# ssheybani/baby-vision-curriculum

Hardware: AMD Instinct MI355X
Metric: video clips/sec (node) VideoMAE-base 16x224^2 bf16 pretraining (higher is better)
Workload: dtype bf16; 1 GPU; VideoMAE-base (ViT-B/16 encoder, 4-layer decoder), 16x224x224 clips, tubelet 2, 90% tube mask, full training step (fwd + MSE + bwd + GradScaler + SGD-Nesterov); clips_per_gpu=256, global_batch=256, parallelism=dp1, weights=random init N(0,0.02), seed 0

## Files before the change

baby-vision-curriculum_amd/_lib.py:

```python
import ctypes
import os
import sys

_HERE = os.path.dirname(os.path.abspath(__file__))
LIB_PATH = os.environ.get("BVC_LIB_PATH") or os.path.join(_HERE, "libbvc_hip.so")

c_void_p, c_int, c_int64, c_float, c_char_p = ctypes.c_void_p, ctypes.c_int, ctypes.c_int64, ctypes.c_float, ctypes.c_char_p
c_double = ctypes.c_double


class BvcError(RuntimeError):
    pass


class VideoMAEConfigC(ctypes.Structure):
    _fields_ = [(n, c_int) for n in (
        "image_size", "patch_size", "num_channels", "num_frames", "tubelet_size",
        "hidden_size", "num_hidden_layers", "num_attention_heads", "intermediate_size",
        "decoder_hidden_size", "decoder_num_hidden_layers", "decoder_num_attention_heads",
        "decoder_intermediate_size")] + [("layer_norm_eps", c_float), ("decoder_norm_eps", c_float),
                                         ("norm_pix_loss", c_int)]


class VitConfigC(ctypes.Structure):
# ... 160 lines not shown
    "bvc_dropout_mask_host": (c_int, [ctypes.c_uint64, ctypes.c_uint64, c_int, c_int, c_int, c_int, c_float, c_void_p]),
    "bvc_videomae_cls_set_drop": (c_int, [c_void_p, ctypes.POINTER(BranchDropC), c_int, c_void_p]),
    "bvc_videomae_encoder_set_drop": (c_int, [c_void_p, ctypes.POINTER(BranchDropC), c_int, c_void_p]),
    "bvc_vit_set_drop": (c_int, [c_void_p, ctypes.POINTER(BranchDropC), c_int, c_void_p]),
    "bvc_predictor_set_drop": (c_int, [c_void_p, ctypes.POINTER(BranchDropC), c_int, c_void_p]),
    "bvc_op_attention_fwd": (c_int, [c_void_p, c_void_p, c_void_p, c_int, c_int, c_int, c_int, c_void_p]),
    "bvc_op_attention_bwd": (c_int, [c_void_p, c_void_p, c_void_p, c_void_p, c_void_p, c_void_p, c_int, c_int, c_int, c_int, c_void_p]),
    "bvc_op_attention_bwd_part": (c_int, [c_void_p, c_void_p, c_void_p, c_void_p, c_void_p, c_void_p, c_int, c_int, c_int, c_int, c_int, c_void_p]),
    "bvc_op_attention_width": (c_int, [c_int]),
    "bvc_op_attention_fwd_scaled": (c_int, [c_void_p, c_void_p, c_void_p, c_int, c_int, c_int, c_int, ctypes.c_float, c_void_p]),
    "bvc_op_attention_bwd_scaled": (c_int, [c_void_p, c_void_p, c_void_p, c_void_p, c_void_p, c_void_p, c_int, c_int, c_int, c_int,
                                            ctypes.c_float, c_void_p]),
    "bvc_op_attention_probs": (c_int, [c_void_p, c_void_p, c_void_p, c_int, c_int, c_int, c_int, ctypes.c_float, c_void_p]),
    "bvc_op_layernorm_fwd": (c_int, [c_void_p, c_int, c_int, c_int, c_void_p, c_void_p, c_void_p, c_void_p, c_void_p,
                                     c_int, c_int, c_float, c_void_p]),
    "bvc_op_layernorm_bwd": (c_int, [c_void_p, c_void_p, c_int, c_int, c_int, c_void_p, c_void_p, c_void_p, c_void_p,
                                     c_int, c_void_p, c_void_p, c_void_p, c_void_p, c_int, c_int, c_void_p]),
    "bvc_op_layernorm_bwd_workspace": (c_int64, [c_int, c_int]),
    "bvc_op_colsum_bf16": (c_int, [c_void_p, c_int, c_int, c_int, c_float, c_void_p, c_void_p, c_void_p]),
    "bvc_op_colsum_f32": (c_int, [c_void_p, c_int, c_int, c_int, c_int, c_int, c_void_p, c_void_p]),
    "bvc_op_cast_bf16": (c_int, [c_void_p, c_void_p, c_int64, c_void_p]),
    "bvc_op_row_normalize": (c_int, [c_void_p, c_void_p, c_void_p, c_int, c_int, c_float, c_void_p]),
    "bvc_op_row_normalize_bwd": (c_int, [c_void_p, c_void_p, c_void_p, c_void_p, c_int, c_int, c_void_p]),
    "bvc_op_nce_finalize": (c_int, [c_void_p, c_int, c_float, c_int64, c_void_p, c_void_p, c_void_p]),
    "bvc_op_sgd_step": (c_int, [c_void_p, c_void_p, c_void_p, c_int64, c_float, c_float, c_float, c_float, c_int, c_int, c_int,
                                c_void_p, c_void_p, c_int, c_void_p, c_void_p]),
    "bvc_videomae_shadow": (c_int, [c_void_p, c_int, ctypes.POINTER(c_void_p), ctypes.POINTER(c_int64)]),
    "bvc_vit_shadow": (c_int, [c_void_p, c_int, ctypes.POINTER(c_void_p), ctypes.POINTER(c_int64)]),
    "bvc_predictor_shadow": (c_int, [c_void_p, c_int, ctypes.POINTER(c_void_p), ctypes.POINTER(c_int64)]),
    "bvc_op_adam_prepare": (c_int, [c_void_p, c_double, c_double, c_double, c_void_p, c_void_p]),
    "bvc_op_adam_step": (c_int, [c_void_p, c_void_p, c_void_p, c_void_p, c_int64, c_double, c_double, c_double, c_double, c_double,
                                 c_int, c_int, c_void_p, c_void_p, c_void_p, c_int, c_void_p, c_void_p]),
    "bvc_op_row_ln_selected": (c_int, [c_int, c_int, c_int, c_int]),
    "bvc_op_sgd_step_segments": (c_int, [c_void_p, c_void_p, c_void_p, c_int64, c_void_p, c_void_p, c_void_p, c_int, c_void_p, c_void_p, c_void_p,
                                         c_int, c_void_p, c_void_p]),
    "bvc_op_adam_step_segments": (c_int, [c_void_p, c_void_p, c_void_p, c_void_p, c_int64, c_void_p, c_void_p, c_void_p, c_int, c_void_p, c_void_p,
                                          c_void_p, c_void_p, c_void_p, c_int, c_void_p, c_void_p]),
    "bvc_op_nonfinite_check": (c_int, [c_void_p, c_int64, c_void_p, c_void_p]),
    "bvc_op_mask_index": (c_int, [c_void_p, c_int, c_int, c_int, c_int, c_void_p, c_void_p, c_void_p, c_void_p]),
    "bvc_op_dual_mask_index": (c_int, [c_void_p, c_void_p, c_int, c_int, c_int, c_int, c_void_p, c_void_p, c_void_p, c_void_p]),
    "bvc_op_gather_patches": (c_int, [c_void_p, c_void_p, c_void_p, c_int, c_int, c_int, c_int, c_int, c_int, c_int, c_int, c_void_p]),
    "bvc_op_pixel_labels": (c_int, [c_void_p, c_void_p, c_void_p, c_int, c_int, c_int, c_int, c_int, c_int, c_int, c_int, c_int, c_void_p]),
    "bvc_comm_unique_id": (c_int, [c_void_p]),
    "bvc_comm_init": (c_int, [c_int, c_int, c_void_p, ctypes.POINTER(c_void_p)]),
    "bvc_comm_destroy": (c_int, [c_void_p]),
    "bvc_comm_stream": (c_void_p, [c_void_p]),
    "bvc_comm_rank": (c_int, [c_void_p]),
    "bvc_comm_world": (c_int, [c_void_p]),
    "bvc_comm_library": (c_char_p, []),
    "bvc_allreduce_bucket": (c_int, [c_void_p, c_void_p, c_int64, c_int, c_void_p]),
    "bvc_comm_wait": (c_int, [c_void_p, c_void_p]),
    "bvc_allgather": (c_int, [c_void_p, c_void_p, c_void_p, c_int64, c_void_p]),
    "bvc_allreduce": (c_int, [c_void_p, c_void_p, c_int64, c_int, c_void_p]),
    "bvc_broadcast": (c_int, [c_void_p, c_void_p, c_int64, c_int, c_void_p]),
}

_lib = None

_det_flag = False
_det_pushed = False


def use_deterministic_algorithms(mode):
    global _det_flag
    _det_flag = bool(mode)
    lib()
# ... 51 lines not shown
```

baby-vision-curriculum_amd/csrc/gemm.h:

```cpp
#pragma once
#include "common.h"
#include "dropgate.h"
#include "../../include/bvc.h"

namespace bvc {

enum GemmLayout { GEMM_NT = BVC_GEMM_NT, GEMM_NN = BVC_GEMM_NN, GEMM_TN = BVC_GEMM_TN };

enum GemmEpilogue {
    EPI_F32 = BVC_EPI_F32,
    EPI_BF16 = BVC_EPI_BF16,
    EPI_GELU = BVC_EPI_GELU,
    EPI_RESID = BVC_EPI_RESID,
    EPI_POS = BVC_EPI_POS,
    EPI_E2D = BVC_EPI_E2D,
    EPI_LOSS = BVC_EPI_LOSS,
    EPI_DGELU = BVC_EPI_DGELU,
    EPI_F32_BF16 = BVC_EPI_F32_BF16,
    EPI_RELU = BVC_EPI_RELU,
    EPI_DRELU = BVC_EPI_DRELU,
    EPI_NCE = BVC_EPI_NCE,
    EPI_NCE_BWD = BVC_EPI_NCE_BWD,
    EPI_RESID_LN = BVC_EPI_RESID_LN,
    EPI_DLN = BVC_EPI_DLN,
    EPI_RESID_GATE = BVC_EPI_RESID_GATE
};

using GemmProblem = bvc_gemm_desc;

constexpr int kMaxGroup = 4;

struct Options { int gemm8 = 0; int dw_overlap = 0; int row_ln = 0; int row_stagger = 1; int deterministic = 0; int head_pad = 0; int dec_tail = 1; };
Options& options();

float* det_scratch(size_t floats, hipStream_t stream);
size_t det_scratch_bytes();
int det_scratch_release();

struct DryRun { bool on = false; char name[160] = ""; };
DryRun& dry_run();

int launch_gemm(const GemmProblem* probs, int nprob, GemmLayout layout, int tile_cfg, hipStream_t stream, int stages = -1);

int launch_gemm_gate(const GemmProblem& p, const Gate& gate, int tile_cfg, hipStream_t stream);

int gemm_num_tiles(const GemmProblem& p, int tile_cfg);
int gemm_pick_tile(const GemmProblem* probs, int nprob, int tile_cfg);
bool gemm_row_ln_ok(int M, int N, int K);
constexpr size_t kRowLnPartFloats = 512 * 2 * 384;

}
```

baby-vision-curriculum_amd/csrc/gemm.hip:

```cpp
#include <stdio.h>
#include <stdlib.h>
#include <string.h>

#include <algorithm>
#include <mutex>
#include <vector>

#include "gemm_tile.h"

namespace bvc {

Options& options() {
    static Options o;
    return o;
}
DryRun& dry_run() {
    static thread_local DryRun d;
    return d;
}

template <int BM, int BN, bool AT, bool BT, int NS, int LB = 2, bool EARLY_ = true>
__global__ __launch_bounds__(256, LB) void gemm_kernel(const GemmGroup g) {
    constexpr bool DET = false;
#include "gemm_kernel_body.inc"
// ... 298 lines not shown
    BVC_REQUIRE(p.A && p.B && p.C && p.resid, "launch_gemm_gate: null operand, output or residual");
    BVC_REQUIRE(gate.rows >= 1 && (double)p.M * p.N < 4398046511104.0, "launch_gemm_gate: bad gate (rows per sample %d) or more than 2^42 elements", gate.rows);
    const int cfg = gemm_pick_tile(&p, 1, tile_cfg);
    GemmGroup g;
    g.nprob = 1;
    g.bal_units = g.bal_lb = g.bal_tiles = 0;
    g.accum = 0;
    g.stagger = 0;
    g.dbg = 0;
    const int total = tiles_for(p, cfg);
    for (int i = 0; i < kMaxGroup; ++i) { g.prob[i] = p; g.panel[i] = pick_panel(p, cfg, GEMM_NT); g.tile_start[i] = i == 0 ? 0 : total; }
    g.tile_start[kMaxGroup] = total;
    switch (cfg) {
        case 0: return launch_gate_one<128, 128>(g, gate, total, stream);
        case 1: return launch_gate_one<128, 64>(g, gate, total, stream);
        default: return launch_gate_one<64, 64>(g, gate, total, stream);
    }
}

int launch_gemm(const GemmProblem* probs, int nprob, GemmLayout layout, int tile_cfg, hipStream_t stream, int stages) {
    BVC_REQUIRE(nprob >= 1 && nprob <= kMaxGroup, "launch_gemm: nprob %d out of range", nprob);
    for (int i = 0; i < nprob; ++i)
        BVC_REQUIRE(probs[i].epi != EPI_RESID_GATE, "launch_gemm: BVC_EPI_RESID_GATE needs its gate (bvc_op_gemm_gate / a context with bvc_*_set_drop)");
    static thread_local bool skip_g8 = false;
    bool auto_g8 = false;
    if (probs[0].epi == EPI_RESID_LN || probs[0].epi == EPI_DLN) {
        const GemmProblem& p = probs[0];
        BVC_REQUIRE(nprob == 1 && (tile_cfg < 0 || tile_cfg == 12), "launch_gemm: the LayerNorm epilogues take one problem on tile config 12");
        BVC_REQUIRE(gemm_row_ln_ok(p.M, p.N, p.K) && p.ldc == p.N && p.split_k == 1 && p.a_bytes < 0x80000000u && p.b_bytes < 0x80000000u,
                    "launch_gemm: the LayerNorm epilogues need N == ldc == 384, K %% 64 == 0, operands below 2 GiB (M=%d N=%d K=%d)", p.M, p.N, p.K);
        BVC_REQUIRE(p.C && p.C2 && p.ln_mean && p.ln_rstd && p.ln_gamma, "launch_gemm: LayerNorm epilogue with a null output / statistic / scale");
        if (p.epi == EPI_RESID_LN) BVC_REQUIRE(layout == GEMM_NT && p.resid && p.ln_beta, "launch_gemm: RESID_LN is an NT product with a residual and a LayerNorm bias");
        if (p.epi == EPI_DLN) BVC_REQUIRE(layout == GEMM_NN && p.ln_x && p.ln_part && p.ln_dgamma && p.ln_dbeta, "launch_gemm: DLN is an NN product with the LayerNorm input, partial scratch and parameter gradients");
        if (p.seg_rows != 0)
            BVC_REQUIRE(p.seg_rows > 0 && p.seg_rows % 128 == 0 && p.M % p.seg_rows == 0 && p.seg_off >= 0 && p.seg_stride > 0 &&
                            (long long)p.seg_off + p.seg_rows <= (long long)p.seg_stride,
                        "launch_gemm: bad segment map (seg_rows %d: a multiple of 128 that divides M = %d; seg_off %d + seg_rows <= seg_stride %d)",
                        p.seg_rows, p.M, p.seg_off, p.seg_stride);
        tile_cfg = 12;
    } else {
        for (int i = 0; i < nprob; ++i)
            BVC_REQUIRE(probs[i].seg_rows == 0, "launch_gemm: a segment map (seg_rows %d) exists for BVC_EPI_RESID_LN / BVC_EPI_DLN only", probs[i].seg_rows);
    }
    if (tile_cfg < 0 && stages < 0 && nprob == 1 && options().gemm8 >= 0 && probs[0].epi == EPI_BF16 && gemm_as_ok(probs[0], layout) &&
        (options().gemm8 > 0 || probs[0].M >= 16384) && BVC_EXP_ENV("BVC_GEMM_NO_AS") == nullptr)
        return launch_gemm_as(probs[0], layout, 0, stream);
    if (tile_cfg < 0 && stages < 0 && !skip_g8) {
        const int g8 = pick_gemm8(probs, nprob, layout);
        if (g8 > 0) { tile_cfg = g8; auto_g8 = true; }
    }
    if (tile_cfg >= 15 && tile_cfg <= 18) {
        BVC_REQUIRE(nprob == 1, "launch_gemm: tile configs 15 - 18 take one problem");
        const int rc = launch_gemm_as(probs[0], layout, tile_cfg - 15, stream);
        BVC_REQUIRE(rc != 1, "launch_gemm: tile configs 15 - 18 (A-stationary kernel) take NT products with K = 384, N %% 128 == 0, BF16 / GELU epilogues");
        return rc;
    }
    if ((tile_cfg >= 3 && tile_cfg <= 5) || tile_cfg == 8) {
#ifdef BVC_EXPERIMENTS
        BVC_REQUIRE(nprob == 1 && layout == GEMM_NT, "launch_gemm: tile configs 3-5 (32-deep K steps) are NT, one problem");
        BVC_REQUIRE(!options().deterministic || probs[0].split_k == 1, "launch_gemm: tile configs 3-5 have no deterministic split-K form");
        return launch_gemm_big_nt(probs[0], tile_cfg, stream);
#else
        BVC_REQUIRE(false, "launch_gemm: tile configs 3-5 / 8 exist only in a -DBVC_EXPERIMENTS build (csrc/experiments/gemm_big.hip)");
#endif
    }
    bool accum = false;
// ... 143 lines not shown
```

baby-vision-curriculum_amd/csrc/gemm8.hip:

```cpp
#include <stdio.h>
#include <stdlib.h>

#include <type_traits>

#include "gemm_tile.h"
#include "rowops.h"

namespace bvc {

namespace {

typedef __attribute__((ext_vector_type(4))) unsigned int u32x4;

#ifndef BVC_G8_ST_AUX
#define BVC_G8_ST_AUX 0
#endif
#ifndef BVC_G8_ROW_ST_AUX
#define BVC_G8_ROW_ST_AUX 0
#endif
constexpr uint32_t kInvalidBase = 0x80000000u;

struct Unit {
    int pi, m0, n0, kt0, nkt, split, tile;
};
// ... 39 lines not shown
        const int w = lid - split * ntiles;
        if (tiles_n > tiles_m) { tm = w % tiles_m; tn = w / tiles_m; } else { tm = w / tiles_n; tn = w % tiles_n; }
    } else {
        split = lid % p.split_k;
        const int tl = lid / p.split_k;
        const bool m_fast = tiles_n > tiles_m;
        tm = m_fast ? tl % tiles_m : tl / tiles_n;
        tn = m_fast ? tl / tiles_m : tl % tiles_n;
    }
    const int nt_all = (p.K + 63) / 64;
    int per = (nt_all + p.split_k - 1) / p.split_k;
    per = (per + 1) & ~1;
    int kt0 = split * per;
    if (g.bal_units > 0) {
        kt0 = split * g.bal_lb;
        per = tail ? (nt_all - kt0 + 1) & ~1 : g.bal_lb;
    }
    u.pi = pi;
    u.m0 = __builtin_amdgcn_readfirstlane(tm * BM);
    u.n0 = __builtin_amdgcn_readfirstlane(tn * BN);
    u.kt0 = __builtin_amdgcn_readfirstlane(kt0);
    u.nkt = __builtin_amdgcn_readfirstlane(per);
    u.split = __builtin_amdgcn_readfirstlane(split);
    u.tile = __builtin_amdgcn_readfirstlane(tm * tiles_n + tn);
}

}

template <int BM, int BN, bool AT, bool BT, int EC>
__global__ __launch_bounds__(512, 1) void gemm8_kernel(const GemmGroup g, const int total_units) {
    extern __shared__ __attribute__((aligned(16))) char smem[];
    static_assert(BM == 256 || (BM == 128 && BN == 384), "128-row tiles: the 128 x 384 geometry only");
    static_assert(BN == 256 || BN == 128 || (BN == 384 && BM == 128), "column tiles of 256 / 128, or 384 with 128 rows");
    static_assert((EC == 4 || EC == 5) == (BM == 128 && !AT), "row epilogues (EC 4 / 5) are the k-contiguous-A instantiations of the 128 x 384 tile, and only they");
    static_assert(BM == 256 || EC == 4 || EC == 5 || (AT && BT && (EC == 2 || EC == 6)), "128 x 384 with transposed A: weight gradients");
    static_assert(EC != 6 || (AT && BT), "EC 6 (deterministic weight gradients) is a TN product");
    static_assert(EC != 4 || !BT, "EC 4 (residual + LayerNorm forward) is an NT product");
    constexpr int A_BYTES = BM * 64 * 2, B_BYTES = BN * 64 * 2, TILE = A_BYTES + B_BYTES;
    constexpr int WMR = BM / 2;
    constexpr int WN = BN / 4, TN = WN / 16, TM = WMR / 16, TMH = TM / 2;
    constexpr int NB = BN / 64, NBH = BN / 128, NAH = BM / 128;
    constexpr int n0c = AT ? NBH : (NB == 6 ? 3 : NB < 2 ? NB : 2), n1c = AT ? NAH : NB - n0c, n2c = AT ? NBH : BM / 128, n3c = AT ? NAH : BM / 128;
    constexpr int RT = BM / 128;
    constexpr int KMAX = (n0c > 2 || n1c > 2 || n2c > 2 || n3c > 2) ? 3 : 2;
    constexpr int PT = n0c + n1c + n2c + n3c;
#ifdef BVC_G8_DMA_LATE
    constexpr bool LATE = true;
#else
    constexpr bool LATE = false;
#endif
    constexpr int PAR_BYTES = EC == 4 ? 3 * BN * 4 : EC == 5 ? BN * 4 : 0, STAT_OFF = PAR_BYTES, COL_OFF = STAT_OFF + 4096;
    constexpr int CPR = BN == 384 ? 8 : WN / 8;
    constexpr int NSIDE = TM * (16 / (64 / CPR));
    static_assert(PT + 2 * NSIDE < 64, "vmcnt is a 6-bit counter");
    constexpr int WP = AT ? PT : n3c + n0c + n1c;
    constexpr int W1 = LATE ? n0c + n1c + n2c : PT;
    constexpr int W3 = LATE ? (AT ? n2c + n3c + n0c : n3c + n0c) : WP;

    const int tid = threadIdx.x, lane = tid & 63;
    const int wave = __builtin_amdgcn_readfirstlane(tid >> 6);
    const int wm = wave >> 2, wn = wave & 3;

    const int xcd = blockIdx.x & 7, slot_id = blockIdx.x >> 3, nslots = gridDim.x >> 3;
    const int xq = total_units >> 3, xr = total_units & 7;
    const int x_lo = xcd < xr ? xcd * (xq + 1) : xr * (xq + 1) + (xcd - xr) * xq;
    const int x_hi = x_lo + xq + (xcd < xr ? 1 : 0);
    int uid = x_lo + slot_id, u_step = nslots, u_hi = x_hi;
    if (EC == 2 && g.bal_units > 0) {
        u_step = 1;
        if (uid < x_hi) {
            u_hi = uid + 1;
        } else {
            const int J = xcd * nslots - x_lo + (uid - x_hi), I = 8 * nslots - g.bal_units;
            uid = g.bal_units + (J * g.bal_tiles) / I;
            u_hi = g.bal_units + ((J + 1) * g.bal_tiles) / I;
        }
    }
    if (uid >= u_hi) {
        if constexpr (EC == 5) {
            float* pr = g.prob[0].ln_part + (size_t)blockIdx.x * 2 * BN;
            for (int i = tid; i < 2 * BN; i += 512) pr[i] = 0.f;
        }
        return;
    }
    if constexpr (EC == 4 || EC == 5) {
        const int cnt = x_hi - x_lo, r = cnt % nslots, nmax = (cnt + nslots - 1) / nslots;
        int num = 0, den = 1;
        if (r > 0 && slot_id >= r) { num = slot_id - r + 1; den = nslots - r + 1; }
        else if (r == 0 && nmax >= 4) { num = slot_id; den = 2 * nslots; }
        const int quanta = __builtin_amdgcn_readfirstlane((int)((long long)g.stagger * num / den));
        for (int i = 0; i < quanta / 127; ++i) __builtin_amdgcn_s_sleep(127);
    }
    if (BVC_DBG(g, 1024) && (slot_id & 1)) {
        for (int i = 0; i < ((g.dbg >> 12) & 63); ++i) __builtin_amdgcn_s_sleep(127);
    }

    Unit su;
    decode_unit<BM, BN>(g, uid, su);
    int s_uid = uid, s_kt = 0;
    bool s_valid = true;
    __amdgpu_buffer_rsrc_t s_ra, s_rb;
    uint32_t s_la, s_lb, s_baseA, s_baseB, s_strideA, s_strideB;
    auto s_problem = [&]() {
        const GemmProblem& p = g.prob[su.pi];
        s_ra = make_rsrc(p.A, p.a_bytes);
        s_rb = make_rsrc(p.B, p.b_bytes);
        if constexpr (!AT) {
            const int r = 8 * wave + (lane >> 3);
            s_la = (uint32_t)((r * p.lda + (((lane & 7) ^ swz_rows(r)) << 3)) * 2);
            s_strideA = (uint32_t)(64 * p.lda * 2);
        } else {
            const int kr = 4 * wave + (lane >> 4);
            s_la = (uint32_t)((kr * p.lda + (((lane & 15) ^ swz_tr<128>(kr)) << 3)) * 2);
            s_strideA = (uint32_t)(32 * p.lda * 2);
        }
        if constexpr (!BT) {
            const int r = 8 * wave + (lane >> 3);
            s_lb = (uint32_t)((r * p.ldb + (((lane & 7) ^ swz_rows(r)) << 3)) * 2);
// ... 57 lines not shown
            else { if constexpr (K < n3c) load_a(ra_, BM == 256 ? (K == 0 ? 1 : 3) : 1); }
        } else {
            if constexpr (GI == 0) { if constexpr (K < NBH) load_b(rb_, 2 * K); }
            else if constexpr (GI == 1) { if constexpr (K < NAH) load_a(ra_, 2 * K); }
            else if constexpr (GI == 2) { if constexpr (K < NBH) load_b(rb_, 2 * K + 1); }
            else { if constexpr (K < NAH) load_a(ra_, 2 * K + 1); }
        }
        if constexpr (GI == 3 && K == KMAX - 1) s_advance();
    };
    auto stage_group = [&](auto gi_, char* buf) {
        stage_one(gi_, I0{}, buf); stage_one(gi_, I1{}, buf);
        if constexpr (KMAX == 3) stage_one(gi_, I2{}, buf);
    };
    auto stage_phase = [&](auto q_, auto k_, char* cur, char* oth) {
        constexpr int Q = decltype(q_)::value;
        if constexpr (Q == 0) stage_one(I2{}, k_, oth);
        else if constexpr (Q == 1) stage_one(I3{}, k_, oth);
        else if constexpr (Q == 2) stage_one(I0{}, k_, cur);
        else stage_one(I1{}, k_, cur);
    };

    char* const buf0 = smem;
    char* const buf1 = smem + TILE;
    constexpr int PARK = BN == 384 ? 16 * 48 * 4 : 16 * WN * 4;
    AS3 char* const wl = (AS3 char*)smem + 2 * TILE + wave * PARK;

    if constexpr (EC == 0) {
        const GemmProblem& p0 = g.prob[0];
        AS3 float* lbias = (AS3 float*)((AS3 char*)smem + 2 * TILE);
        const int npad = ((p0.N + BN - 1) / BN) * BN;
        for (int i = tid; i < npad; i += 512) lbias[i] = (p0.bias && i < p0.N) ? p0.bias[i] : 0.f;
        __syncthreads();
    }
    if constexpr (EC == 4 || EC == 5) {
        const GemmProblem& p0 = g.prob[0];
        AS3 float* lpar = (AS3 float*)((AS3 char*)smem + 2 * TILE);
        for (int i = tid; i < BN; i += 512) {
            if constexpr (EC == 4) {
                lpar[i] = p0.bias ? p0.bias[i] : 0.f;
                lpar[BN + i] = p0.ln_gamma[i];
                lpar[2 * BN + i] = p0.ln_beta[i];
            } else {
                lpar[i] = p0.ln_gamma[i];
            }
        }
        if constexpr (EC == 5) {
            AS3 float* lcol = (AS3 float*)((AS3 char*)smem + 2 * TILE + COL_OFF);
            for (int i = tid; i < 8 * 2 * WN; i += 512) lcol[i] = 0.f;
        }
        __syncthreads();
    }
    s_problem();
    s_ktile();
    stage_group(I0{}, buf0); stage_group(I1{}, buf0); stage_group(I2{}, buf0); stage_group(I3{}, buf0);
    stage_group(I0{}, buf1); stage_group(I1{}, buf1);
    wait_vmcnt<WP>();
    asm volatile("s_barrier" ::: "memory");
#ifndef BVC_G8_NO_STAGGER
    if (wm == 1) asm volatile("s_barrier" ::: "memory");
#endif

    Unit cu;
    decode_unit<BM, BN>(g, uid, cu);
    int after_epi = 0;


    while (true) {
        const GemmProblem& p = g.prob[cu.pi];
        f32x4 acc[TM][TN];
#pragma unroll
        for (int i = 0; i < TM; ++i)
#pragma unroll
            for (int j = 0; j < TN; ++j) acc[i][j] = f32x4{0.f, 0.f, 0.f, 0.f};
        float rsum[2] = {0.f, 0.f};
        const bool do_rowsum = (EC == 2 || EC == 6) && p.rowsum != nullptr && cu.n0 == 0;

        auto ktile = [&](auto rs_, char* cur, char* oth) {
            constexpr bool RS = decltype(rs_)::value;
            const char* la = cur;
            const char* lb = cur + A_BYTES;
            if constexpr (!AT) {
// ... 95 lines not shown
                                case 2: a = af[2]; break;
                                default: a = af[3]; break;
                            }
                        } else {
                            a = wn == 0 ? af[0] : af[1];
                        }
                        union { bf16x8 v; uint32_t u[4]; } w;
                        w.v = a;
                        float t0 = 0.f, t1 = 0.f;
#pragma unroll
                        for (int e = 0; e < 4; ++e) {
                            t0 += __uint_as_float(w.u[e] << 16);
                            t1 += __uint_as_float(w.u[e] & 0xffff0000u);
                        }
                        rsum[mh] += t0 + t1;
                    }
                    __builtin_amdgcn_s_setprio(0);
                    __builtin_amdgcn_sched_barrier(0);
                    asm volatile("s_barrier" ::: "memory");
                };
                phase(I0{}); phase(I1{}); phase(I2{}); phase(I3{});
            }
            after_epi = 0;
        };

        for (int kt = 0; kt < cu.nkt; kt += 2) {
            ktile(std::bool_constant<EC == 2 || EC == 6>{}, buf0, buf1);
            ktile(std::bool_constant<EC == 2 || EC == 6>{}, buf1, buf0);
        }

        const int m0 = cu.m0, n0 = cu.n0;
        const int epi = p.epi, Mrows = p.M, Ncols = p.N, ldc = p.ldc;
        int seg_shift = 0;
        if constexpr (EC == 4 || EC == 5) {
            if (p.seg_rows > 0) {
                const int upc = p.seg_rows >> 7, u = m0 >> 7, c = u / upc;
                seg_shift = __builtin_amdgcn_readfirstlane(c * p.seg_stride + p.seg_off + ((u - c * upc) << 7) - m0);
            }
        }
        const float alpha = p.alpha_dev ? p.alpha * p.alpha_dev[0] : p.alpha;
        constexpr int UNITS = WN / 4;
        constexpr int RPU = 64 / CPR;
        constexpr int U = 16 / RPU;
        static_assert(NSIDE == TM * U, "epilogue geometry");
        int nstores = 0;
        constexpr uint32_t kDrop = 0xFFFFFFF0u;
        auto park = [&](int i) {
            const int row = lane & 15;
#pragma unroll
            for (int j = 0; j < TN; ++j) {
                const int unit = (4 * j + (lane >> 4)) ^ (row & (UNITS - 1));
                *reinterpret_cast<AS3 f32x4*>(wl + row * (WN * 4) + unit * 16) = acc[i][j];
            }
        };
        const bool atomic = p.split_k > 1 || g.accum != 0;
        if constexpr (EC == 0) {
            const __amdgpu_buffer_rsrc_t rc = make_rsrc(p.C, BVC_DBG(g, 1) ? 0u : kDrop);
            const __amdgpu_buffer_rsrc_t rc2 = make_rsrc(p.C2 ? p.C2 : p.C, BVC_DBG(g, 1) ? 0u : kDrop);
            const AS3 float* lbias = (const AS3 float*)((AS3 char*)smem + 2 * TILE);
            const int q4 = lane >> 4;
            f32x4 bj[TN];
#pragma unroll
            for (int j = 0; j < TN; ++j) {
                const int nb = n0 + wn * WN + 16 * j + 4 * q4;
                bj[j] = *reinterpret_cast<const AS3 f32x4*>(lbias + nb);
            }
            const bool two_out = epi == EPI_GELU;
// ... 85 lines not shown
            issue(I0{});
            wait_vmcnt<0>();
#pragma unroll
            for (int j = 0; j < TN; ++j) asm volatile("" : "+v"(rs[0][j]));
            tile(I0{}); tile(I1{}); tile(I2{}); tile(I3{});
            asm volatile("s_waitcnt lgkmcnt(0)\n\ts_barrier" ::: "memory");
#pragma unroll
            for (int i = 0; i < TM; ++i) {
                asm volatile("" ::: "memory");
                const AS3 f32x4* sp = reinterpret_cast<const AS3 f32x4*>(lstat + (wm * 64 + 16 * i + r16) * 8);
                const f32x4 a = sp[0], b = sp[1];
                const float mean = ((a[0] + a[2]) + (b[0] + b[2])) * (1.f / BN);
                const float d0 = a[0] * (1.f / WN) - mean, d1 = a[2] * (1.f / WN) - mean, d2 = b[0] * (1.f / WN) - mean, d3 = b[2] * (1.f / WN) - mean;
                const float m2 = ((a[1] + a[3]) + (b[1] + b[3])) + (float)WN * ((d0 * d0 + d1 * d1) + (d2 * d2 + d3 * d3));
                const float rstd = rsqrtf(m2 * (1.f / BN) + eps);
                const int m = m0 + 32 * i + 16 * wm + r16;
                if (wn == 0 && q4 == 0) {
                    __builtin_amdgcn_raw_buffer_store_b32(__float_as_uint(mean), rmu, (uint32_t)m * 4u, 0, 0);
                    __builtin_amdgcn_raw_buffer_store_b32(__float_as_uint(rstd), rrs, (uint32_t)m * 4u, 0, 0);
                }
                const uint32_t o2 = ((uint32_t)m * (uint32_t)BN + (uint32_t)(wn * WN + 16 * (q4 & 1) + 8 * (q4 >> 1))) * 2u;
#pragma unroll
                for (int jp = 0; jp < TN / 2; ++jp) {
                    const f32x4 ga = *reinterpret_cast<const AS3 f32x4*>(lpar + BN + cw + 32 * jp), gb = *reinterpret_cast<const AS3 f32x4*>(lpar + BN + cw + 32 * jp + 16);
                    const f32x4 ba = *reinterpret_cast<const AS3 f32x4*>(lpar + 2 * BN + cw + 32 * jp), bb = *reinterpret_cast<const AS3 f32x4*>(lpar + 2 * BN + cw + 32 * jp + 16);
                    const f32x4 ya = ((acc[i][2 * jp] - mean) * rstd) * ga + ba;
                    const f32x4 yb = ((acc[i][2 * jp + 1] - mean) * rstd) * gb + bb;
                    const uint32_t a0 = pack2bf(ya[0], ya[1]), a1 = pack2bf(ya[2], ya[3]), b0 = pack2bf(yb[0], yb[1]), b1 = pack2bf(yb[2], yb[3]);
                    const auto s0 = __builtin_amdgcn_permlane16_swap(a0, b0, false, false);
                    const auto s1 = __builtin_amdgcn_permlane16_swap(a1, b1, false, false);
                    __builtin_amdgcn_raw_buffer_store_b128(u32x4{s0[0], s1[0], s0[1], s1[1]}, rc2, o2 + 64u * jp, 0, BVC_G8_ROW_ST_AUX);
                }
            }
        } else if constexpr (EC == 5) {
            const uint32_t ext = (uint32_t)Mrows * (uint32_t)(BN * 4);
            const __amdgpu_buffer_rsrc_t rx = make_rsrc(p.ln_x, ext), rd = make_rsrc(reinterpret_cast<float*>(p.C) + (size_t)seg_shift * BN, ext), rc2 = make_rsrc(p.C2, ext / 2);
            const __amdgpu_buffer_rsrc_t rmu = make_rsrc(p.ln_mean, (uint32_t)Mrows * 4u), rrs = make_rsrc(p.ln_rstd, (uint32_t)Mrows * 4u);
            const AS3 float* lpar = (const AS3 float*)((AS3 char*)smem + 2 * TILE);
            AS3 float* lstat = (AS3 float*)((AS3 char*)smem + 2 * TILE + STAT_OFF);
            AS3 float* lcol = (AS3 float*)((AS3 char*)smem + 2 * TILE + COL_OFF) + wave * 2 * WN;
            const int q4 = lane >> 4, r16 = lane & 15;
            const int cw = wn * WN + 4 * q4;
            const int mrow = m0 + 16 * wm + r16;
            const uint32_t obase = (uint32_t)mrow * (uint32_t)(BN * 4) + (uint32_t)cw * 4u;
            const uint32_t o2base = ((uint32_t)mrow * (uint32_t)BN + (uint32_t)(wn * WN + 16 * (q4 & 1) + 8 * (q4 >> 1))) * 2u;
            f32x4 xr[2][TN], dr[TN];
            float mu[2], rsd[2];
            auto issue = [&](auto i_) {
                constexpr int i = decltype(i_)::value;
                mu[i & 1] = __uint_as_float(__builtin_amdgcn_raw_buffer_load_b32(rmu, (uint32_t)(mrow + 32 * i) * 4u, 0, 0));
                rsd[i & 1] = __uint_as_float(__builtin_amdgcn_raw_buffer_load_b32(rrs, (uint32_t)(mrow + 32 * i) * 4u, 0, 0));
#pragma unroll
                for (int j = 0; j < TN; ++j)
                    xr[i & 1][j] = __builtin_bit_cast(f32x4, __builtin_amdgcn_raw_buffer_load_b128(rx, obase + (uint32_t)(i * 32 * BN * 4 + 64 * j), 0, 0));
            };
            auto tile = [&](auto i_) {
                constexpr int i = decltype(i_)::value, b = i & 1;
                __builtin_amdgcn_sched_barrier(0);
#pragma unroll
                for (int j = 0; j < TN; ++j)
                    dr[j] = __builtin_bit_cast(f32x4, __builtin_amdgcn_raw_buffer_load_b128(rd, obase + (uint32_t)(i * 32 * BN * 4 + 64 * j), 0, 0));
                if constexpr (i + 1 < TM) issue(std::integral_constant<int, i + 1>{});
                __builtin_amdgcn_sched_barrier(0);
                float s1 = 0.f, s2 = 0.f;
#pragma unroll
                for (int j = 0; j < TN; ++j) {
                    const f32x4 gam = *reinterpret_cast<const AS3 f32x4*>(lpar + cw + 16 * j);
                    const f32x4 gv = acc[i][j] * alpha;
                    const f32x4 xh = (xr[b][j] - mu[b]) * rsd[b];
                    const f32x4 gg = gv * gam;
                    f32x4 tg = gv * xh, tb = gv;
                    s1 += (gg[0] + gg[1]) + (gg[2] + gg[3]);
                    const f32x4 gx = gg * xh;
                    s2 += (gx[0] + gx[1]) + (gx[2] + gx[3]);
                    xr[b][j] = xh;
                    acc[i][j] = gg;
#pragma unroll
                    for (int e = 0; e < 4; ++e) {
                        tg[e] = row16_sum(tg[e]);
                        tb[e] = row16_sum(tb[e]);
                    }
                    if (r16 == 0) {
                        AS3 f32x4* cg = reinterpret_cast<AS3 f32x4*>(lcol + 16 * j + 4 * q4);
                        AS3 f32x4* cb = reinterpret_cast<AS3 f32x4*>(lcol + WN + 16 * j + 4 * q4);
                        *cg = *cg + tg;
                        *cb = *cb + tb;
                    }
                }
                s1 += __shfl_xor(s1, 16, 64);
                s1 += __shfl_xor(s1, 32, 64);
                s2 += __shfl_xor(s2, 16, 64);
                s2 += __shfl_xor(s2, 32, 64);
                if (q4 == 0) *reinterpret_cast<AS3 f32x2*>(lstat + ((wm * 64 + 16 * i + r16) * 4 + wn) * 2) = f32x2{s1, s2};
                asm volatile("s_waitcnt lgkmcnt(0)\n\ts_barrier" ::: "memory");
                const AS3 f32x4* sp = reinterpret_cast<const AS3 f32x4*>(lstat + (wm * 64 + 16 * i + r16) * 8);
                const f32x4 sa = sp[0], sb = sp[1];
                const float c1 = ((sa[0] + sa[2]) + (sb[0] + sb[2])) * (1.f / BN), c2 = ((sa[1] + sa[3]) + (sb[1] + sb[3])) * (1.f / BN);
#pragma unroll
                for (int j = 0; j < TN; ++j) {
                    acc[i][j] = ((acc[i][j] - c1) - xr[b][j] * c2) * rsd[b] + dr[j];
                    __builtin_amdgcn_raw_buffer_store_b128(__builtin_bit_cast(u32x4, acc[i][j]), rd, obase + (uint32_t)(i * 32 * BN * 4 + 64 * j), 0, BVC_G8_ROW_ST_AUX);
                }
#pragma unroll
                for (int jp = 0; jp < TN / 2; ++jp) {
                    const f32x4 ya = acc[i][2 * jp], yb = acc[i][2 * jp + 1];
                    const uint32_t a0 = pack2bf(ya[0], ya[1]), a1 = pack2bf(ya[2], ya[3]), b0 = pack2bf(yb[0], yb[1]), b1 = pack2bf(yb[2], yb[3]);
                    const auto w0 = __builtin_amdgcn_permlane16_swap(a0, b0, false, false);
                    const auto w1 = __builtin_amdgcn_permlane16_swap(a1, b1, false, false);
                    __builtin_amdgcn_raw_buffer_store_b128(u32x4{w0[0], w1[0], w0[1], w1[1]}, rc2, o2base + (uint32_t)(i * 32 * BN * 2 + 64 * jp), 0, BVC_G8_ROW_ST_AUX);
                }
            };
            issue(I0{});
            wait_vmcnt<0>();
            asm volatile("" : "+v"(mu[0]), "+v"(rsd[0]));
#pragma unroll
            for (int j = 0; j < TN; ++j) asm volatile("" : "+v"(xr[0][j]));
            tile(I0{}); tile(I1{}); tile(I2{}); tile(I3{});
        } else if constexpr (BN == 384) {
            const __amdgpu_buffer_rsrc_t rca = make_rsrc(p.C, kDrop);
            const __amdgpu_buffer_rsrc_t rsl = make_rsrc(EC == 6 && atomic ? p.partial + (size_t)cu.split * Mrows * Ncols : p.C, kDrop);
#pragma unroll
            for (int i = 0; i < TM; ++i) {
#pragma unroll
                for (int ps = 0; ps < 2; ++ps) {
                    const int prow = lane & 15;
#pragma unroll
                    for (int jj = 0; jj < 3; ++jj)
                        *reinterpret_cast<AS3 f32x4*>(wl + prow * 192 + (4 * jj + (lane >> 4)) * 16) = acc[i][3 * ps + jj];
#pragma unroll
                    for (int t = 0; t < 16 * 48 / 64; ++t) {
                        const int idx = t * 64 + lane;
                        const int row = idx / 48, col = idx % 48;
                        const int m = m0 + wm * WMR + 16 * i + row, n = n0 + wn * WN + 48 * ps + col;
                        const float v = *reinterpret_cast<const AS3 float*>(wl + row * 192 + col * 4) * alpha;
// ... 154 lines not shown
            }
            }
            if (EC == 1 && epi == EPI_LOSS) {
                const float w = wave_sum(sumsq);
                float* red = reinterpret_cast<float*>(smem + 2 * TILE);
                if (lane == 0) red[wave * (16 * WN)] = w;
                asm volatile("s_waitcnt lgkmcnt(0)\n\ts_barrier" ::: "memory");
                asm volatile("s_barrier" ::: "memory");
                if (tid == 0) {
                    float s = 0.f;
#pragma unroll
                    for (int q = 0; q < 8; ++q) s += red[q * (16 * WN)];
                    p.partial[cu.tile] = s;
                }
            }
        }
        if (do_rowsum) {
#pragma unroll
            for (int mh = 0; mh < 2; ++mh) {
                float v = rsum[mh];
                v += __shfl_xor(v, 16, 64);
                v += __shfl_xor(v, 32, 64);
                const int m = m0 + wm * WMR + 16 * (TMH * mh + wn) + lane;
                if constexpr (EC == 6) {
                    if (wn < TMH && (lane >> 4) == 0 && m < p.M) p.ln_part[(size_t)cu.split * p.M + m] = v * alpha;
                } else {
                    if (wn < TMH && (lane >> 4) == 0 && m < p.M) atomicAdd(p.rowsum + m, v * alpha);
                }
            }
        }
        uid += u_step;
        if (uid >= u_hi) break;
        decode_unit<BM, BN>(g, uid, cu);
        after_epi = (EC == 4 || EC == 5) ? -1 : (((EC == 2 || EC == 6) && atomic) || BN == 384) ? 0 : EC == 0 ? nstores : -1;
    }
    wait_vmcnt<0>();
#ifndef BVC_G8_NO_STAGGER
    if (wm == 0) asm volatile("s_barrier" ::: "memory");
#endif
    if constexpr (EC == 5) {
        __syncthreads();
        const AS3 float* lcol = (const AS3 float*)((AS3 char*)smem + 2 * TILE + COL_OFF);
        float* pr = g.prob[0].ln_part + (size_t)blockIdx.x * 2 * BN;
        for (int c = tid; c < 2 * BN; c += 512) {
            const int which = c / BN, col = c % BN, w = col / WN, cc = col % WN;
            pr[c] = lcol[(w * 2 + which) * WN + cc] + lcol[((4 + w) * 2 + which) * WN + cc];
        }
    }
}

static int g8_ncu() {
    static int ncu = 0;
    if (ncu == 0) {
        int dev = 0;
        hipDeviceProp_t prop;
        if (hipGetDevice(&dev) != hipSuccess || hipGetDeviceProperties(&prop, dev) != hipSuccess) return 256;
        ncu = prop.multiProcessorCount > 0 ? (prop.multiProcessorCount / 8) * 8 : 256;
        if (ncu < 8) ncu = 8;
    }
    return ncu;
}

static bool plan_balance(GemmGroup& g, int bm, int bn, int total, int ncu) {
    if (BVC_EXP_ENV("BVC_G8_NO_BALANCE") != nullptr) return false;
    const int S = g.prob[0].split_k, nt = (g.prob[0].K + 63) / 64;
    if ((S < 2 && !g.accum) || total >= ncu || total % S != 0) return false;
    for (int i = 0; i < g.nprob; ++i) {
        const GemmProblem& p = g.prob[i];
        if (p.split_k != S || (p.K + 63) / 64 != nt || p.epi != EPI_F32) return false;
        if (g.tile_start[i] % S != 0 || g.panel[i] == 0) return false;
    }
    const int T = total / S, I = ncu - total, q = (T + I - 1) / I;
    double e = 6.0, c = 1.0;
    if (const char* v = BVC_EXP_ENV("BVC_G8_BALANCE_EPI")) e = atof(v);
    if (const char* v = BVC_EXP_ENV("BVC_G8_BALANCE_TAIL")) c = atof(v);
    const double lt = ((double)nt / S - (q - 1) * e) / (q * c + 1.0 / S);
    if (lt < 2.0) return false;
    const int per = (((nt + S - 1) / S) + 1) & ~1;
    const int lb = (int)((nt - lt) / S) & ~1;
    if (lb < 8 || nt - S * lb < 2 || lb > 0.95 * per) return false;
    g.bal_units = total;
    g.bal_lb = lb;
    g.bal_tiles = T;
    (void)bm; (void)bn;
    return true;
}

template <int BM, int BN, bool AT, bool BT, int EC>
static int launch_gemm8_one(const GemmGroup& g_in, int total, hipStream_t stream) {
    constexpr size_t lds = 2 * (size_t)(BM + BN) * 64 * 2 + (EC == 0 ? (size_t)32768 : EC == 4 ? (size_t)(3 * BN * 4 + 4096) : EC == 5 ? (size_t)(BN * 4 + 4096 + 8 * 2 * (BN / 4) * 4) :
                                                              BN == 384 ? (size_t)8 * 16 * 48 * 4 : (size_t)8 * 16 * (BN / 4) * 4);
    static_assert(lds <= 160 * 1024, "LDS per CU");
    if (dry_run().on) {
        snprintf(dry_run().name, sizeof(dry_run().name), "bvc::gemm8_kernel<%d, %d, %s, %s, %d>", BM, BN, AT ? "true" : "false", BT ? "true" : "false", EC);
        return BVC_OK;
    }
    static bool attr_set = false;
    if (!attr_set) {
        BVC_CHECK_HIP(hipFuncSetAttribute(reinterpret_cast<const void*>(&gemm8_kernel<BM, BN, AT, BT, EC>),
                                          hipFuncAttributeMaxDynamicSharedMemorySize, (int)lds));
        attr_set = true;
    }
    const int ncu = g8_ncu();
    GemmGroup g = g_in;
    int grid = total < ncu ? ((total + 7) / 8) * 8 : ncu;
    if constexpr (EC == 2) {
        if (plan_balance(g, BM, BN, total, ncu)) grid = ncu;
    }
    if constexpr (EC == 4 || EC == 5) {
        const double us = 1.45 * ((g.prob[0].K + 63) / 64) + (EC == 4 ? 23.0 : 32.0);
        g.stagger = options().row_stagger && total > ncu ? (int)(us * 33.0) : 0;
    }
    hipLaunchKernelGGL((gemm8_kernel<BM, BN, AT, BT, EC>), dim3(grid), dim3(512), lds, stream, g, total);
    BVC_CHECK_HIP(hipGetLastError());
    (void)0;
    if constexpr (EC == 5)
        return launch_ln_param_reduce(g.prob[0].ln_part, grid, BN, g.prob[0].ln_dgamma, g.prob[0].ln_dbeta, stream);
    return BVC_OK;
}

static int epi_class(int epi, GemmLayout layout) {
    if (layout == GEMM_TN) return epi == EPI_F32 ? 2 : -1;
    if (epi == EPI_RESID_LN) return layout == GEMM_NT ? 4 : -1;
    if (epi == EPI_DLN) return layout == GEMM_NN ? 5 : -1;
    switch (epi) {
        case EPI_BF16: case EPI_GELU: case EPI_RELU: return 0;
        case EPI_DGELU: case EPI_DRELU: return 3;
        case EPI_F32: case EPI_RESID: case EPI_POS: case EPI_E2D: case EPI_LOSS: case EPI_F32_BF16: return 1;
        default: return -1;
    }
}

int launch_gemm8(const GemmGroup& g, GemmLayout layout, int bn, hipStream_t stream, bool det) {
    const int total = g.tile_start[g.nprob];
    int ec = -2;
    for (int i = 0; i < g.nprob; ++i) {
        const GemmProblem& p = g.prob[i];
        const int c = epi_class(p.epi, layout);
        if (c < 0 || (ec != -2 && c != ec)) return 1;
        ec = c;
        if (p.a_bytes >= kInvalidBase || p.b_bytes >= kInvalidBase) return 1;
        if (layout != GEMM_TN && (p.split_k != 1 || p.K % 64 != 0)) return 1;
        if (layout == GEMM_TN && p.split_k > 1 && p.epi != EPI_F32) return 1;
        if (p.rowsum && layout != GEMM_TN) return 1;
        if (c == 0 && (g.nprob != 1 || (size_t)((p.N + bn - 1) / bn) * bn * 4 > (size_t)32768)) return 1;
    }
    if (total <= 0) return 1;
#define BVC_G8(BN_, AT_, BT_, EC_) return launch_gemm8_one<256, BN_, AT_, BT_, EC_>(g, total, stream)
    if (bn == 384) {
        if (layout == GEMM_TN) return ec != 2 ? 1 : det ? launch_gemm8_one<128, 384, true, true, 6>(g, total, stream)
                                                        : launch_gemm8_one<128, 384, true, true, 2>(g, total, stream);
        const GemmProblem& p = g.prob[0];
        if (g.nprob != 1 || p.N != 384 || p.ldc != 384 || (double)p.M * 1536.0 >= 4294000000.0) return 1;
        if (ec == 4 && layout == GEMM_NT) return launch_gemm8_one<128, 384, false, false, 4>(g, total, stream);
        if (ec == 5 && layout == GEMM_NN) return launch_gemm8_one<128, 384, false, true, 5>(g, total, stream);
        return 1;
    }
    if (ec >= 4) return 1;
    if (layout == GEMM_NT) {
        if (ec == 0) { if (bn == 256) BVC_G8(256, false, false, 0); else BVC_G8(128, false, false, 0); }
        if (ec == 3) { if (bn == 256) BVC_G8(256, false, false, 3); else BVC_G8(128, false, false, 3); }
        if (ec == 1) { if (bn == 256) BVC_G8(256, false, false, 1); else BVC_G8(128, false, false, 1); }
    } else if (layout == GEMM_NN) {
        if (ec == 0) { if (bn == 256) BVC_G8(256, false, true, 0); else BVC_G8(128, false, true, 0); }
        if (ec == 3) { if (bn == 256) BVC_G8(256, false, true, 3); else BVC_G8(128, false, true, 3); }
        if (ec == 1) { if (bn == 256) BVC_G8(256, false, true, 1); else BVC_G8(128, false, true, 1); }
    } else if (det) {
        if (bn == 256) BVC_G8(256, true, true, 6); else BVC_G8(128, true, true, 6);
    } else {
        if (bn == 256) BVC_G8(256, true, true, 2); else BVC_G8(128, true, true, 2);
    }
#undef BVC_G8
    return 1;
}

}
```

baby-vision-curriculum_amd/csrc/rowops.h:

```cpp
#pragma once
#include "common.h"
#include "dropgate.h"

namespace bvc {

struct RowMap { int rin, rout, roff; };
static inline RowMap identity_rows() { return RowMap{0, 0, 0}; }

struct PatchGeom { int T, C, H, W, ts, ps; };

struct PixelSrc {
    const void* ptr;
    int is_u8;
    float mean[4], stdv[4];
};
static inline PixelSrc pixels_f32(const float* p) { return PixelSrc{p, 0, {0, 0, 0, 0}, {1, 1, 1, 1}}; }

int launch_ln_fwd(const float* x, RowMap rm, const float* gamma, const float* beta, bf16_t* y, float* mean, float* rstd,
                  int M, int D, float eps, hipStream_t s, float* y32 = nullptr);
size_t ln_bwd_workspace_floats(int M, int D);
size_t ln_bwd_workspace_floats_upto(int Mmax, int D);
int launch_ln_bwd(const bf16_t* dy, const float* x, RowMap rm, const float* mean, const float* rstd, const float* gamma,
                  float* dres, int accumulate, bf16_t* dres_bf, float* dgamma, float* dbeta, float* part, int M, int D, hipStream_t s,
                  const Gate* gate = nullptr,
                  bool compact_x = false);
int launch_ln_param_reduce(const float* part, int nblk, int D, float* dgamma, float* dbeta, hipStream_t s);
int launch_colsum_bf16(const bf16_t* X, int M, int N, int ld, float alpha, float* out, hipStream_t s);
int launch_colsum_bf16_scaled(const bf16_t* X, int M, int N, int ld, float alpha, const float* alpha_dev, float* out, hipStream_t s);
int launch_colsum_f32(const float* X, RowMap rm, int M, int D, float* out, hipStream_t s);
int launch_token_mean(const float* x, int B, int N, int D, float* out, hipStream_t s);
int launch_token_mean_bwd(const float* dmean, int B, int N, int D, float* dx, hipStream_t s);
int launch_fcnorm_bwd_bcast(const float* dy, const float* p, const float* mean, const float* rstd, const float* gamma, float* dres,
                            bf16_t* dres_bf, float* dgamma, float* dbeta, int B, int N, int D, hipStream_t s, const Gate* gate = nullptr);
int launch_dropout_mask(const Gate& gate, size_t n, uint8_t* out, hipStream_t s);
void dropout_mask_host(const Gate& gate, size_t n, uint8_t* out);
int launch_cast_bf16(const float* in, bf16_t* out, size_t n, hipStream_t s);
int launch_gather_rows_bf16(const float* in, RowMap rm, bf16_t* out, int M, int D, hipStream_t s);
int launch_mask_index(const uint8_t* mask, int B, int L, int nvis, int nmask, int* vis_idx, int* msk_idx, int* status, hipStream_t s);
int launch_dual_mask_index(const uint8_t* mask, const uint8_t* decode, int B, int L, int nvis, int ndec, int* vis_idx, int* dec_idx,
                           int* status, hipStream_t s);
int launch_gather_patches(PixelSrc clip, const int* vis_idx, bf16_t* A, int B, int nvis, PatchGeom pg, hipStream_t s);
int launch_labels(PixelSrc clip, const int* dec_idx, float* labels, int B, int ndec, PatchGeom pg, int norm_pix, hipStream_t s);
int launch_fill_masked(float* xfull, const float* mask_token, const float* pos, const int* dec_idx, int B, int Ld, int nvis,
                       int ndec, int D, hipStream_t s);
int launch_sgd_step(float* p, float* g, float* buf, size_t n, float lr, float momentum, float dampening, float wd, int nesterov,
                    int first, int maximize, const float* grad_scale, const float* found_inf, int write_grad, bf16_t* shadow,
                    hipStream_t s);
int launch_adam_prep(float* state, double lr, double beta1, double beta2, const float* found_inf, hipStream_t s);
int launch_adam_step(float* p, float* g, float* m, float* v, size_t n, double lr, double beta1, double beta2, double eps, double wd,
                     int decoupled, int maximize, const float* state, const float* grad_scale, const float* found_inf, int write_grad,
                     bf16_t* shadow, hipStream_t s);
int launch_sgd_step_segments(float* p, float* g, float* buf, int64_t n, const int64_t* seg_start, const int* seg_group, const int* blk_seg,
                             int nseg, const bvc_sgd_groups* groups, const float* grad_scale, const float* found_inf, int write_grad,
                             bf16_t* shadow, hipStream_t s);
int launch_adam_step_segments(float* p, float* g, float* m, float* v, int64_t n, const int64_t* seg_start, const int* seg_group,
                              const int* blk_seg, int nseg, const bvc_adam_groups* groups, float* state, double* hyper_dev,
                              const float* grad_scale, const float* found_inf, int write_grad, bf16_t* shadow, hipStream_t s);
int launch_pad_heads(const bf16_t* wqkv, const float* bqkv, const bf16_t* wo, bf16_t* wqkv_p, float* bqkv_p, bf16_t* wo_p, int D, int H,
                     int hd, int hdp, hipStream_t s);
int launch_unpad_head_grads(const float* gwqkv_p, const float* gbqkv_p, const float* gwo_p, float* gwqkv, float* gbqkv, float* gwo, int D,
                            int H, int hd, int hdp, hipStream_t s);
int launch_nonfinite_check(const float* x, size_t n, float* found_inf, hipStream_t s);
int launch_row_normalize(const float* f, bf16_t* fn, float* inv, int n, int p, float eps, hipStream_t s);
int launch_row_normalize_bwd(const float* f, const float* inv, const float* dfn, float* df, int n, int p, hipStream_t s);
int launch_nce_finalize(const float* partial, int ntiles, float inv_t, double npos, float* loss, float* stats, hipStream_t s);
int launch_target_select(const float* h, const int* idx, float* out, int nsets, int B, int Np, int L, int D, float eps, hipStream_t s);
int launch_pred_assemble(const float* xe, const float* mask_token, const float* pos, const int* idx_pred, float* X, int nsets, int B,
                         int Nc, int Np, int D, hipStream_t s);
int launch_pred_ctx_grad(const float* dX, bf16_t* dxe, int nsets, int B, int Nc, int Np, int D, hipStream_t s);
int smooth_l1_blocks(size_t n);
int launch_smooth_l1_fwd(const float* z, const float* h, size_t n, float* partial, float* loss, hipStream_t s);
int launch_smooth_l1_bwd(const float* z, const float* h, const float* gout, size_t n, float* dz, hipStream_t s);
int launch_ema(float* k, const float* q, size_t n, float m, hipStream_t s);
int launch_iota_mod(int* idx, int n, int L, hipStream_t s);
int launch_loss_finalize(const float* partial, int n, double count, const int* status, float* loss, hipStream_t s);

}
// ... 1 lines not shown
```

baby-vision-curriculum_amd/csrc/rowops.hip:

```cpp
#include "rowops.h"
#include "gemm.h"

#include <algorithm>

namespace bvc {

constexpr int kMaxChunks = 4;
constexpr int kWideChunks = 6;

__device__ __forceinline__ int map_row(int m, RowMap rm) {
    return rm.rin > 0 ? (m / rm.rin) * rm.rout + rm.roff + (m % rm.rin) : m;
}

template <int LPR>
__device__ __forceinline__ float row_sum(float v) {
#pragma unroll
    for (int o = LPR / 2; o > 0; o >>= 1) v += __shfl_xor(v, o, 64);
    return v;
}

template <int LPR, int NC>
__global__ __launch_bounds__(256) void ln_fwd_kernel(const float* __restrict__ x, RowMap rm, const float* __restrict__ gamma,
                                                     const float* __restrict__ beta, bf16_t* __restrict__ y, float* __restrict__ y32,
                                                     float* __restrict__ mean, float* __restrict__ rstd, int M, int D, float eps) {
// ... 231 lines not shown
    const int lane = threadIdx.x & 63, wave = threadIdx.x >> 6;
    const int col = (blockIdx.x * 64 + lane) * 8;
    float acc[8] = {0, 0, 0, 0, 0, 0, 0, 0};
    const int r0 = blockIdx.y * RB, r1 = min(M, r0 + RB);
    if (col < N) {
        for (int m = r0 + wave; m < r1; m += 4) {
            const bf16x8 v = *reinterpret_cast<const bf16x8*>(X + (size_t)m * ld + col);
#pragma unroll
            for (int e = 0; e < 8; ++e) acc[e] += bf2f((bf16_t)v[e]);
        }
    }
#pragma unroll
    for (int e = 0; e < 8; ++e) red[wave][lane * 8 + e] = acc[e];
    __syncthreads();
    for (int c = threadIdx.x; c < 512; c += 256) {
        const int n = blockIdx.x * 512 + c;
        if (n < N) {
            const float v = (alpha_dev ? alpha * alpha_dev[0] : alpha) * ((red[0][c] + red[1][c]) + (red[2][c] + red[3][c]));
            if constexpr (DET) out[(size_t)blockIdx.y * N + n] = v;
            else atomicAdd(out + n, v);
        }
    }
}
__global__ __launch_bounds__(256) void colsum_bf16_kernel(const bf16_t* __restrict__ X, int M, int N, int ld, float alpha,
                                                          const float* __restrict__ alpha_dev, float* __restrict__ out, int RB) {
    colsum_bf16_body<false>(X, M, N, ld, alpha, alpha_dev, out, RB);
}
__global__ __launch_bounds__(256) void colsum_bf16_det_kernel(const bf16_t* __restrict__ X, int M, int N, int ld, float alpha,
                                                              const float* __restrict__ alpha_dev, float* __restrict__ part, int RB) {
    colsum_bf16_body<true>(X, M, N, ld, alpha, alpha_dev, part, RB);
}

template <bool DET>
__device__ __forceinline__ void colsum_f32_body(const float* __restrict__ X, RowMap rm, int M, int D, float* __restrict__ out, int RB) {
    __shared__ float red[4][256];
    const int lane = threadIdx.x & 63, wave = threadIdx.x >> 6;
    const int col = (blockIdx.x * 64 + lane) * 4;
    f32x4 acc = {0, 0, 0, 0};
    const int r0 = blockIdx.y * RB, r1 = min(M, r0 + RB);
    if (col < D)
        for (int m = r0 + wave; m < r1; m += 4)
            acc += *reinterpret_cast<const f32x4*>(X + (size_t)map_row(m, rm) * D + col);
#pragma unroll
    for (int e = 0; e < 4; ++e) red[wave][lane * 4 + e] = acc[e];
    __syncthreads();
    const int c = threadIdx.x;
    const int n = blockIdx.x * 256 + c;
    if constexpr (DET) {
        if (n < D) out[(size_t)blockIdx.y * D + n] = (red[0][c] + red[1][c]) + (red[2][c] + red[3][c]);
    } else {
        if (n < D) atomicAdd(out + n, (red[0][c] + red[1][c]) + (red[2][c] + red[3][c]));
    }
}
__global__ __launch_bounds__(256) void colsum_f32_kernel(const float* __restrict__ X, RowMap rm, int M, int D,
                                                         float* __restrict__ out, int RB) {
    colsum_f32_body<false>(X, rm, M, D, out, RB);
}
__global__ __launch_bounds__(256) void colsum_f32_det_kernel(const float* __restrict__ X, RowMap rm, int M, int D,
                                                             float* __restrict__ part, int RB) {
    colsum_f32_body<true>(X, rm, M, D, part, RB);
}

__global__ __launch_bounds__(256) void token_mean_kernel(const float* __restrict__ x, int N, int D, float* __restrict__ out) {
    __shared__ float red[16][64];
    const int cg = threadIdx.x & 15, rp = threadIdx.x >> 4;
    const int col = blockIdx.x * 64 + cg * 4;
    const float* xb = x + (size_t)blockIdx.y * N * D;
    f32x4 acc = {0, 0, 0, 0};
    if (col < D)
        for (int m = rp; m < N; m += 16) acc += *reinterpret_cast<const f32x4*>(xb + (size_t)m * D + col);
#pragma unroll
    for (int e = 0; e < 4; ++e) red[rp][cg * 4 + e] = acc[e];
    __syncthreads();
    if (threadIdx.x < 64) {
        float t = 0.f;
#pragma unroll
        for (int r = 0; r < 16; ++r) t += red[r][threadIdx.x];
        const int n = blockIdx.x * 64 + threadIdx.x;
        if (n < D) out[(size_t)blockIdx.y * D + n] = t / (float)N;
    }
}

__global__ void token_mean_bwd_kernel(const float* __restrict__ dmean, float* __restrict__ dx, int N, int D, size_t total4) {
    const size_t i = (size_t)blockIdx.x * blockDim.x + threadIdx.x;
    if (i >= total4) return;
    const size_t e = i * 4;
    const int d = (int)(e % D);
    const size_t b = e / ((size_t)N * D);
    f32x4 g = *reinterpret_cast<const f32x4*>(dmean + b * D + d);
    const float inv = 1.f / (float)N;
    g *= inv;
    *reinterpret_cast<f32x4*>(dx + e) = g;
}
// ... 332 lines not shown
#pragma unroll
    for (int i = 0; i < 3; ++i) {
        const int c = l3 + i;
        mr[i] = (c == 0 || c == 3) ? mu[0] : (c == 1 || c == 4) ? mu[1] : mu[2];
        rr[i] = (c == 0 || c == 3) ? rinv[0] : (c == 1 || c == 4) ? rinv[1] : rinv[2];
    }
    __builtin_amdgcn_fence(__ATOMIC_RELEASE, "wavefront");
    __builtin_amdgcn_wave_barrier();
    __builtin_amdgcn_fence(__ATOMIC_ACQUIRE, "wavefront");
    float* out = labels + (size_t)m * CE;
#pragma unroll
    for (int k = 0; k < CE / 256; ++k) {
        const int o = lane * 4 + 256 * k;
        f32x4 r;
#pragma unroll
        for (int j = 0; j < 4; ++j) {
            const int t = o + j, e = t / 3, c = t - 3 * e;
            r[j] = (buf[c * E + e] - mr[(k + j) % 3]) * rr[(k + j) % 3];
        }
        *reinterpret_cast<f32x4*>(out + o) = r;
    }
}

__global__ void fill_masked_kernel(float* __restrict__ xfull, const float* __restrict__ mask_token, const float* __restrict__ pos,
                                   const int* __restrict__ dec_idx, int B, int Ld, int nvis, int ndec, int D) {
    const size_t i = (size_t)blockIdx.x * blockDim.x + threadIdx.x;
    const int nch = D >> 2;
    if (i >= (size_t)B * ndec * nch) return;
    const int m = (int)(i / nch), c = (int)(i % nch);
    const int b = m / ndec, j = m % ndec;
    const f32x4 mt = reinterpret_cast<const f32x4*>(mask_token)[c];
    const f32x4 pe = reinterpret_cast<const f32x4*>(pos + (size_t)dec_idx[m] * D)[c];
    reinterpret_cast<f32x4*>(xfull + ((size_t)b * Ld + nvis + j) * D)[c] = mt + pe;
}

__global__ __launch_bounds__(256) void loss_finalize_kernel(const float* __restrict__ partial, int n, double count,
                                                            const int* __restrict__ status, float* __restrict__ loss) {
    __shared__ double red[256];
    double s = 0.0;
    for (int i = threadIdx.x; i < n; i += 256) s += (double)partial[i];
    red[threadIdx.x] = s;
    __syncthreads();
    for (int o = 128; o > 0; o >>= 1) {
        if (threadIdx.x < o) red[threadIdx.x] += red[threadIdx.x + o];
        __syncthreads();
    }
    if (threadIdx.x == 0) *loss = (status && *status) ? __int_as_float(0x7fc00000) : (float)(red[0] / count);
}

template <int NC>
__global__ __launch_bounds__(256) void target_select_kernel(const float* __restrict__ h, const int* __restrict__ idx,
                                                            float* __restrict__ out, int rows, int B, int Np, int L, int D, float eps) {
    const int lane = threadIdx.x & 63, m = blockIdx.x * 4 + (threadIdx.x >> 6);
    if (m >= rows) return;
    const int b = (m / Np) % B;
    const f32x4* xr = reinterpret_cast<const f32x4*>(h + ((size_t)b * L + idx[m]) * D);
    const int nch = D >> 2;
    f32x4 v[NC];
    float s = 0.f;
#pragma unroll
    for (int i = 0; i < NC; ++i) {
        const int c = lane + 64 * i;
        if (c < nch) { v[i] = xr[c]; s += (v[i][0] + v[i][1]) + (v[i][2] + v[i][3]); }
    }
    const float mu = wave_sum(s) / D;
    float q = 0.f;
// ... 523 lines not shown
        float* mid = nullptr;
        if (const size_t f = det_rows_mid_floats(nblk, 2 * D)) {
            mid = det_scratch(f, s);
            if (!mid) return BVC_ERR_HIP;
        }
        return launch_det_rows_reduce(part, nblk, 2 * D, D, dgamma, dbeta, mid, s);
    }
    hipLaunchKernelGGL(ln_param_reduce_kernel, dim3((2 * D + 255) / 256, (nblk + 15) / 16), dim3(256), 0, s, part, nblk, D, dgamma, dbeta);
    BVC_CHECK_HIP(hipGetLastError());
    return BVC_OK;
}

int launch_colsum_bf16_scaled(const bf16_t* X, int M, int N, int ld, float alpha, const float* alpha_dev, float* out, hipStream_t s) {
    BVC_REQUIRE(N % 8 == 0 && ld % 8 == 0, "colsum_bf16: N and ld must be multiples of 8");
    const int RB = M >= 16384 ? 256 : 64;
    if (options().deterministic) {
        const int nrb = (M + RB - 1) / RB;
        if (nrb <= 0) return BVC_OK;
        float* part = det_scratch((size_t)nrb * N + det_rows_mid_floats(nrb, N), s);
        if (!part) return BVC_ERR_HIP;
        hipLaunchKernelGGL(colsum_bf16_det_kernel, dim3((N + 511) / 512, nrb), dim3(256), 0, s, X, M, N, ld, alpha, alpha_dev, part, RB);
        BVC_CHECK_HIP(hipGetLastError());
        return launch_det_rows_reduce(part, nrb, N, N, out, out, part + (size_t)nrb * N, s);
    }
    hipLaunchKernelGGL(colsum_bf16_kernel, dim3((N + 511) / 512, (M + RB - 1) / RB), dim3(256), 0, s, X, M, N, ld, alpha, alpha_dev, out, RB);
    BVC_CHECK_HIP(hipGetLastError());
    return BVC_OK;
}

int launch_colsum_bf16(const bf16_t* X, int M, int N, int ld, float alpha, float* out, hipStream_t s) {
    return launch_colsum_bf16_scaled(X, M, N, ld, alpha, nullptr, out, s);
}

int launch_colsum_f32(const float* X, RowMap rm, int M, int D, float* out, hipStream_t s) {
    BVC_REQUIRE(D % 4 == 0, "colsum_f32: D must be a multiple of 4");
    const int RB = 256;
    if (options().deterministic) {
        const int nrb = (M + RB - 1) / RB;
        if (nrb <= 0) return BVC_OK;
        float* part = det_scratch((size_t)nrb * D + det_rows_mid_floats(nrb, D), s);
        if (!part) return BVC_ERR_HIP;
        hipLaunchKernelGGL(colsum_f32_det_kernel, dim3((D + 255) / 256, nrb), dim3(256), 0, s, X, rm, M, D, part, RB);
        BVC_CHECK_HIP(hipGetLastError());
        return launch_det_rows_reduce(part, nrb, D, D, out, out, part + (size_t)nrb * D, s);
    }
    hipLaunchKernelGGL(colsum_f32_kernel, dim3((D + 255) / 256, (M + RB - 1) / RB), dim3(256), 0, s, X, rm, M, D, out, RB);
    BVC_CHECK_HIP(hipGetLastError());
    return BVC_OK;
}

int launch_token_mean(const float* x, int B, int N, int D, float* out, hipStream_t s) {
    BVC_REQUIRE(D % 4 == 0, "token_mean: D must be a multiple of 4");
    hipLaunchKernelGGL(token_mean_kernel, dim3((D + 63) / 64, B), dim3(256), 0, s, x, N, D, out);
    BVC_CHECK_HIP(hipGetLastError());
    return BVC_OK;
}

int launch_token_mean_bwd(const float* dmean, int B, int N, int D, float* dx, hipStream_t s) {
    BVC_REQUIRE(D % 4 == 0, "token_mean_bwd: D must be a multiple of 4");
    const size_t total4 = (size_t)B * N * D / 4;
    hipLaunchKernelGGL(token_mean_bwd_kernel, dim3(blocks_for(total4)), dim3(256), 0, s, dmean, dx, N, D, total4);
    BVC_CHECK_HIP(hipGetLastError());
    return BVC_OK;
}

int launch_dropout_mask(const Gate& gate, size_t n, uint8_t* out, hipStream_t s) {
    BVC_REQUIRE(out && n > 0 && (double)n < 4398046511104.0, "dropout_mask: bad argument");
    hipLaunchKernelGGL(dropout_mask_kernel, dim3(blocks_for((n + 3) / 4)), dim3(256), 0, s, gate, n, out);
    BVC_CHECK_HIP(hipGetLastError());
    return BVC_OK;
}

void dropout_mask_host(const Gate& gate, size_t n, uint8_t* out) {
    for (size_t q = 0; q * 4 < n; ++q) {
        uint32_t r[4];
        gate_draws(gate, q, r);
        for (int e = 0; e < 4 && q * 4 + e < n; ++e) out[q * 4 + e] = r[e] >= gate.thr ? 1 : 0;
    }
}
// ... 59 lines not shown
    BVC_REQUIRE(pg.ps % 4 == 0, "labels: patch size must be a multiple of 4");
    const int E = pg.ts * pg.ps * pg.ps;
    const size_t lds = (size_t)(pg.C * E + 2 * pg.C) * 4;
    const int nchunk = pg.C * (E >> 2), ntok = B * ndec;
    if (pg.C == 3 && (E == 512 || E == 256)) {
        const int nblk = (ntok + 3) / 4;
        if (E == 512) hipLaunchKernelGGL(labels_wave3_kernel<2>, dim3(nblk), dim3(256), (size_t)4 * 3 * E * 4, s, clip, dec_idx, labels, ntok, ndec, pg, norm_pix);
        else hipLaunchKernelGGL(labels_wave3_kernel<1>, dim3(nblk), dim3(256), (size_t)4 * 3 * E * 4, s, clip, dec_idx, labels, ntok, ndec, pg, norm_pix);
        BVC_CHECK_HIP(hipGetLastError());
        return BVC_OK;
    }
    if (nchunk <= 512 && lds <= 16384) {
        const int per_wave = (pg.C * E + 2 * pg.C + 3) & ~3;
        const int nblk = (ntok + 3) / 4;
        if (nchunk <= 384)
            hipLaunchKernelGGL(labels_wave_kernel<6>, dim3(nblk), dim3(256), (size_t)per_wave * 16, s, clip, dec_idx, labels, ntok, ndec, pg, norm_pix);
        else
            hipLaunchKernelGGL(labels_wave_kernel<8>, dim3(nblk), dim3(256), (size_t)per_wave * 16, s, clip, dec_idx, labels, ntok, ndec, pg, norm_pix);
        BVC_CHECK_HIP(hipGetLastError());
        return BVC_OK;
    }
    hipLaunchKernelGGL(labels_kernel, dim3(B * ndec), dim3(256), lds, s, clip, dec_idx, labels, ndec, pg, norm_pix);
    BVC_CHECK_HIP(hipGetLastError());
    return BVC_OK;
}

int launch_fill_masked(float* xfull, const float* mask_token, const float* pos, const int* dec_idx, int B, int Ld, int nvis,
                       int ndec, int D, hipStream_t s) {
    hipLaunchKernelGGL(fill_masked_kernel, dim3(blocks_for((size_t)B * ndec * (D / 4))), dim3(256), 0, s, xfull, mask_token, pos, dec_idx, B, Ld, nvis, ndec, D);
    BVC_CHECK_HIP(hipGetLastError());
    return BVC_OK;
}

int launch_target_select(const float* h, const int* idx, float* out, int nsets, int B, int Np, int L, int D, float eps, hipStream_t s) {
    BVC_REQUIRE(D % 4 == 0 && D <= kWideChunks * 256, "target_select: D=%d unsupported", D);
    const int rows = nsets * B * Np;
    if (D > kMaxChunks * 256)
        hipLaunchKernelGGL(target_select_kernel<kWideChunks>, dim3((rows + 3) / 4), dim3(256), 0, s, h, idx, out, rows, B, Np, L, D, eps);
    else
        hipLaunchKernelGGL(target_select_kernel<kMaxChunks>, dim3((rows + 3) / 4), dim3(256), 0, s, h, idx, out, rows, B, Np, L, D, eps);
    BVC_CHECK_HIP(hipGetLastError());
    return BVC_OK;
}

int launch_pred_assemble(const float* xe, const float* mask_token, const float* pos, const int* idx_pred, float* X, int nsets, int B,
                         int Nc, int Np, int D, hipStream_t s) {
    const size_t items = (size_t)nsets * B * (Nc + Np) * (D / 4);
    hipLaunchKernelGGL(pred_assemble_kernel, dim3(blocks_for(items)), dim3(256), 0, s, xe, mask_token, pos, idx_pred, X, nsets * B, B, Nc, Np, D);
    BVC_CHECK_HIP(hipGetLastError());
    return BVC_OK;
}

int launch_pred_ctx_grad(const float* dX, bf16_t* dxe, int nsets, int B, int Nc, int Np, int D, hipStream_t s) {
    hipLaunchKernelGGL(pred_ctx_grad_kernel, dim3(blocks_for((size_t)B * Nc * (D / 4))), dim3(256), 0, s, dX, dxe, nsets, B, Nc, Np, D);
    BVC_CHECK_HIP(hipGetLastError());
    return BVC_OK;
}

int smooth_l1_blocks(size_t n) { return (int)std::min<size_t>(1024, (n + 1023) / 1024); }

int launch_smooth_l1_fwd(const float* z, const float* h, size_t n, float* partial, float* loss, hipStream_t s) {
    BVC_REQUIRE(n > 0, "smooth_l1: empty input");
    const int nb = smooth_l1_blocks(n);
    hipLaunchKernelGGL(smooth_l1_fwd_kernel, dim3(nb), dim3(256), 0, s, z, h, n, partial);
    BVC_CHECK_HIP(hipGetLastError());
    return launch_loss_finalize(partial, nb, (double)n, nullptr, loss, s);
// ... 162 lines not shown
```

baby-vision-curriculum_amd/csrc/stack.h:

```cpp
#pragma once
#include <string>
#include <vector>

#include "attention.h"
#include "gemm.h"
#include "rowops.h"

namespace bvc {

#define TRY(expr)                      \
    do {                               \
        int _rc = (expr);              \
        if (_rc != BVC_OK) return _rc; \
    } while (0)

struct LayerOff {
    int64_t ln1w, ln1b, wqkv, bqkv, wo, bo, ln2w, ln2b, w1, b1, w2, b2, end;
};

struct ParamEntry {
    std::string name;
    int64_t offset, numel;
    int ndim;
    int64_t shape[5];
// ... 40 lines not shown
        *p = reinterpret_cast<T*>(q);
        return BVC_OK;
    }
    void release() {
        for (void* p : ptrs) (void)hipFree(p);
        ptrs.clear();
    }
};

struct Work {
    const float* params = nullptr;
    const bf16_t* wbf = nullptr;
    bf16_t *dyb[3] = {}, *dhb[2] = {}, *dqkv[2] = {}, *dh[2] = {};
    bf16_t *dln = nullptr, *dctx = nullptr;
    float *delta = nullptr, *ln_part = nullptr;
    hipStream_t side = nullptr;
    hipEvent_t ev_fork = nullptr, ev_join[2] = {nullptr, nullptr};
    bool overlap = false;
    int seq = 0;
    bool join_pending[2] = {false, false};
    int64_t pend_lo[2], pend_hi[2];
    const DropState* drop = nullptr;
    int drop_layer = -1;
};

inline int attn_width(int hd) {
    if ((hd == 80 || hd == 88) && !options().head_pad) return hd;
    return hd <= 32 ? 32 : hd <= 64 ? 64 : hd <= 96 ? 96 : 128;
}

struct LayerTail { int nvis, ndec; };
bool layer_tail_ok(const Work& w, const Stack& s, int B, int nvis, int ndec);

LayerOff add_layer_params(ParamTable& t, const std::string& prefix, int64_t d, int64_t inter, bool hf_names);
int alloc_stack(Arena& a, Stack& s, int D, int I, int H, int nlayers, float eps, size_t M, size_t BHN);
int alloc_work(Arena& a, Work& w, size_t MD, size_t MI, size_t delta_elems, size_t lnpart_elems);
void free_work(Work& w);

GemmProblem gemm(const bf16_t* A, size_t a_elems, int lda, const bf16_t* B, size_t b_elems, int ldb, int M, int N, int K,
                 int epi, void* C, int ldc);
int plan_dw(GemmProblem* g, int n);
int join_side(Work& w, int parity, hipStream_t st, bvc_bucket_fn on_bucket, void* user);
void begin_backward(Work& w);
int layer_forward(Work& w, Stack& s, int li, const LayerOff& o, const float* x_in, float* x_out, int B, int N, hipStream_t st,
                  const LayerOff* next = nullptr, const LayerTail* tail = nullptr);
bool fuse_row_ln(const Stack& s, int M);
int set_drop(DropState& d, const bvc_branch_drop* drop, int samples, const char* who, hipStream_t st);
int alloc_drop(Arena& a, DropState& d, int nlayers, int max_samples);
int take_drop(DropState& d, int samples, int rows, const char* who);
inline const Gate* top_gate(const DropState& d, Gate& store) {
    if (!d.active) return nullptr;
    store = d.gate(d.nlayers - 1, 1);
    return &store;
}
int layer_backward(Work& w, Stack& s, int li, const LayerOff& o, const float* x_in, float* dres, float* G, int B, int N,
                   hipStream_t st, bvc_bucket_fn on_bucket, void* user, const LayerTail* tail = nullptr);

}
```

baby-vision-curriculum_amd/csrc/stack.hip:

```cpp
#include <math.h>
#include <stdlib.h>
#include <string.h>

#include <algorithm>

#include "stack.h"

namespace bvc {

int64_t ParamTable::add(const std::string& name, std::initializer_list<int64_t> shp) {
    ParamEntry e;
    e.name = name;
    e.offset = total;
    e.numel = 1;
    e.ndim = (int)shp.size();
    int i = 0;
    for (auto s : shp) { e.shape[i++] = s; e.numel *= s; }
    for (; i < 5; ++i) e.shape[i] = 1;
    entries.push_back(e);
    total += e.numel;
    return e.offset;
}

LayerOff add_layer_params(ParamTable& t, const std::string& p, int64_t d, int64_t inter, bool hf_names) {
// ... 166 lines not shown
            }
        }
    }
    const int cap = std::max(1, std::min(12, ksteps / 8));
    int tile = 2, split = 1;
    for (int t = 0; t < 3; ++t) {
        int tiles = 0;
        for (int i = 0; i < n; ++i) tiles += ((g[i].M + bm[t] - 1) / bm[t]) * ((g[i].N + bn[t] - 1) / bn[t]);
        const int s = std::max(1, std::min(cap, (480 + tiles / 2) / tiles));
        tile = t; split = s;
        if (tiles * s >= 400) break;
    }
    for (int i = 0; i < n; ++i) g[i].split_k = split;
    return tile;
}

bool fuse_row_ln(const Stack& s, int M) {
    const int mode = options().row_ln;
    if (mode < 0 || options().gemm8 < 0) return false;
    if (!gemm_row_ln_ok(M, s.D, s.D) || s.I % 64 != 0 || (3 * s.Da) % 64 != 0) return false;
    if ((size_t)M * std::max<size_t>(3 * (size_t)s.Da, (size_t)s.I) * 2 >= 0x80000000ull) return false;
    if (mode > 0 || options().gemm8 > 0) return true;
    return M >= 128 * 128;
}

bool layer_tail_ok(const Work& w, const Stack& s, int B, int nvis, int ndec) {
    if (!options().dec_tail || nvis < 1 || ndec < 128 || ndec % 128 != 0) return false;
    if (w.drop != nullptr && w.drop->active) return false;
    if (s.hdp != s.hd || !attn_window_ok(s.hd)) return false;
    if (nvis + ndec <= 160) return false;
    return fuse_row_ln(s, B * (nvis + ndec)) && gemm_row_ln_ok(B * ndec, s.D, s.D);
}

int alloc_drop(Arena& a, DropState& d, int nlayers, int max_samples) {
    d.nlayers = nlayers;
    d.max_samples = max_samples;
    return a.alloc(&d.path_scale, (size_t)nlayers * 2 * max_samples);
}

int set_drop(DropState& d, const bvc_branch_drop* drop, int samples, const char* who, hipStream_t st) {
    d.armed = false;
    if (!drop || (drop->hidden_p == 0.f && drop->path_scale == nullptr)) return BVC_OK;
    BVC_REQUIRE(drop->hidden_p >= 0.f && drop->hidden_p < 1.f, "%s: hidden_p %g outside [0, 1)", who, (double)drop->hidden_p);
    BVC_REQUIRE(samples >= 1 && samples <= d.max_samples, "%s: %d samples outside [1, %d]", who, samples, d.max_samples);
    BVC_REQUIRE(drop->rows_per_sample >= 1, "%s: rows_per_sample must be >= 1", who);
    d.hidden_p = drop->hidden_p;
    d.seed = drop->seed;
    d.offset = drop->offset;
    d.samples = samples;
    d.rows = drop->rows_per_sample;
    d.has_path = drop->path_scale != nullptr;
    if (d.has_path)
        BVC_CHECK_HIP(hipMemcpyAsync(d.path_scale, drop->path_scale, (size_t)d.nlayers * 2 * samples * sizeof(float), hipMemcpyDeviceToDevice, st));
    d.armed = true;
    return BVC_OK;
}

int take_drop(DropState& d, int samples, int rows, const char* who) {
    d.active = d.armed;
    d.armed = false;
    if (!d.active) return BVC_OK;
    if (d.samples != samples || d.rows != rows) {
        d.active = false;
        set_error("%s: the gate was set for %d samples of %d rows, the call has %d of %d", who, d.samples, d.rows, samples, rows);
        return BVC_ERR_INVALID;
    }
    return BVC_OK;
}

int layer_forward(Work& w, Stack& s, int li, const LayerOff& o, const float* x_in, float* x_out, int B, int N, hipStream_t st,
                  const LayerOff* next, const LayerTail* tail) {
    LayerAct& a = s.act[li];
    const int D = s.D, I = s.I, M = B * N;
    const int Mq = tail ? B * tail->ndec : M;
    if (tail) BVC_REQUIRE(next == nullptr && tail->nvis + tail->ndec == N && layer_tail_ok(w, s, B, tail->nvis, tail->ndec), "layer_forward: tail mode is not available for this layer");
    const float* P = w.params;
    const bf16_t* W = w.wbf;
    const float eps = s.eps;
    const bool gated = w.drop != nullptr && w.drop->active;
    const int gl = w.drop_layer >= 0 ? w.drop_layer : li;
    const bool fuse = !gated && fuse_row_ln(s, M);
    if (li == 0) s.ln1_ready = false;
    if (!(fuse && s.ln1_ready)) TRY(launch_ln_fwd(x_in, identity_rows(), P + o.ln1w, P + o.ln1b, a.ln1o, a.mean1, a.rstd1, M, D, eps, st));
    s.ln1_ready = false;
    const int Da = s.Da;
    const bool pad = s.hdp != s.hd;
    const bf16_t *Wqkv = W + o.wqkv, *Wo = W + o.wo;
    const float* bqkv = P + o.bqkv;
    const float sm_scale = pad ? 1.0f / sqrtf((float)s.hd) : 0.f;
    if (pad) {
        TRY(launch_pad_heads(W + o.wqkv, P + o.bqkv, W + o.wo, s.wqkv_pad, s.bqkv_pad, s.wo_pad, D, s.H, s.hd, s.hdp, st));
        Wqkv = s.wqkv_pad; Wo = s.wo_pad; bqkv = s.bqkv_pad;
    }
    {
        GemmProblem p = gemm(a.ln1o, (size_t)M * D, D, Wqkv, (size_t)3 * Da * D, D, M, 3 * Da, D, EPI_BF16, a.qkv, 3 * Da);
        p.bias = bqkv;
        TRY(launch_gemm(&p, 1, GEMM_NT, -1, st));
    }
    if (tail) TRY(launch_attn_fwd_win(a.qkv, a.ctx, a.lse, B, N, s.H, s.hdp, tail->nvis, tail->ndec, st, sm_scale));
    else TRY(launch_attn_fwd(a.qkv, a.ctx, a.lse, B, N, s.H, s.hdp, st, sm_scale));
    {
        GemmProblem p = gemm(a.ctx, (size_t)Mq * Da, Da, Wo, (size_t)D * Da, Da, Mq, D, Da, fuse ? EPI_RESID_LN : EPI_RESID, a.h, D);
        p.bias = P + o.bo; p.resid = x_in;
        if (fuse) { p.C2 = a.ln2o; p.ln_gamma = P + o.ln2w; p.ln_beta = P + o.ln2b; p.ln_mean = a.mean2; p.ln_rstd = a.rstd2; p.ln_eps = eps; }
        if (tail) { p.seg_rows = tail->ndec; p.seg_stride = N; p.seg_off = tail->nvis; }
        if (gated) TRY(launch_gemm_gate(p, w.drop->gate(gl, 0), -1, st));
        else TRY(launch_gemm(&p, 1, GEMM_NT, -1, st));
    }
    if (!fuse) TRY(launch_ln_fwd(a.h, identity_rows(), P + o.ln2w, P + o.ln2b, a.ln2o, a.mean2, a.rstd2, M, D, eps, st));
    {
        GemmProblem p = gemm(a.ln2o, (size_t)Mq * D, D, W + o.w1, (size_t)I * D, D, Mq, I, D, EPI_GELU, a.pre, I);
        p.bias = P + o.b1; p.C2 = a.act;
        TRY(launch_gemm(&p, 1, GEMM_NT, -1, st));
    }
    {
        const bool fuse_next = fuse && next != nullptr && li + 1 < (int)s.act.size();
        GemmProblem p = gemm(a.act, (size_t)Mq * I, I, W + o.w2, (size_t)D * I, I, Mq, D, I, fuse_next ? EPI_RESID_LN : EPI_RESID, x_out, D);
        p.bias = P + o.b2; p.resid = a.h;
        if (fuse_next) {
            LayerAct& an = s.act[li + 1];
            p.C2 = an.ln1o; p.ln_gamma = P + next->ln1w; p.ln_beta = P + next->ln1b; p.ln_mean = an.mean1; p.ln_rstd = an.rstd1; p.ln_eps = eps;
        }
        if (gated) TRY(launch_gemm_gate(p, w.drop->gate(gl, 1), -1, st));
        else TRY(launch_gemm(&p, 1, GEMM_NT, -1, st));
        s.ln1_ready = fuse_next;
    }
    return BVC_OK;
}

int join_side(Work& c_, int parity, hipStream_t st, bvc_bucket_fn on_bucket, void* user) {
    if (!c_.join_pending[parity]) return BVC_OK;
    BVC_CHECK_HIP(hipStreamWaitEvent(st, c_.ev_join[parity], 0));
    c_.join_pending[parity] = false;
    if (on_bucket) on_bucket(c_.pend_lo[parity], c_.pend_hi[parity] - c_.pend_lo[parity], user);
    return BVC_OK;
}

int layer_backward(Work& c_, Stack& s, int li, const LayerOff& o, const float* x_in, float* dres, float* G, int B, int N,
                   hipStream_t st, bvc_bucket_fn on_bucket, void* user, const LayerTail* tail) {
    LayerAct& a = s.act[li];
    const int D = s.D, I = s.I, M = B * N;
    const int Mq = tail ? B * tail->ndec : M;
    const float* P = c_.params;
    const bf16_t* W = c_.wbf;
    const int q = c_.seq, par = q & 1;
    bf16_t* dyb = c_.dyb[q % 3];
    bf16_t* dyb_next = c_.dyb[(q + 1) % 3];
    bf16_t *dh = c_.dh[par], *dhb = c_.dhb[par], *dqkv = c_.dqkv[par];
    TRY(join_side(c_, par, st, on_bucket, user));
    {
        GemmProblem p = gemm(dyb, (size_t)Mq * D, D, W + o.w2, (size_t)D * I, I, Mq, I, D, EPI_DGELU, dh, I);
        p.aux = a.pre; p.ldaux = I;
        TRY(launch_gemm(&p, 1, GEMM_NN, -1, st));
    }
    const bool gated = c_.drop != nullptr && c_.drop->active;
    Gate g_attn, g_below;
    if (gated) { g_attn = c_.drop->gate(li, 0); if (li > 0) g_below = c_.drop->gate(li - 1, 1); }
    const bool fuse = !gated && fuse_row_ln(s, M);
    if (tail) BVC_REQUIRE(fuse && tail->nvis + tail->ndec == N, "layer_backward: tail mode needs the row-LayerNorm epilogues");
    if (fuse) {
        GemmProblem p = gemm(dh, (size_t)Mq * I, I, W + o.w1, (size_t)I * D, D, Mq, D, I, EPI_DLN, dres, D);
        p.C2 = dhb; p.ln_x = a.h; p.ln_mean = a.mean2; p.ln_rstd = a.rstd2; p.ln_gamma = P + o.ln2w;
        p.ln_part = c_.ln_part; p.ln_dgamma = G + o.ln2w; p.ln_dbeta = G + o.ln2b;
        if (tail) { p.seg_rows = tail->ndec; p.seg_stride = N; p.seg_off = tail->nvis; }
        TRY(launch_gemm(&p, 1, GEMM_NN, -1, st));
    } else {
        GemmProblem p = gemm(dh, (size_t)M * I, I, W + o.w1, (size_t)I * D, D, M, D, I, EPI_BF16, c_.dln, D);
        TRY(launch_gemm(&p, 1, GEMM_NN, -1, st));
        TRY(launch_ln_bwd(c_.dln, a.h, identity_rows(), a.mean2, a.rstd2, P + o.ln2w, dres, 1, dhb, G + o.ln2w, G + o.ln2b, c_.ln_part, M, D, st,
                          gated ? &g_attn : nullptr));
    }
    const int Da = s.Da;
    const bool pad = s.hdp != s.hd;
    const bf16_t *Wqkv = W + o.wqkv, *Wo = W + o.wo;
    const float sm_scale = pad ? 1.0f / sqrtf((float)s.hd) : 0.f;
    if (pad) {
        TRY(launch_pad_heads(W + o.wqkv, P + o.bqkv, W + o.wo, s.wqkv_pad, s.bqkv_pad, s.wo_pad, D, s.H, s.hd, s.hdp, st));
        Wqkv = s.wqkv_pad; Wo = s.wo_pad;
    }
    {
        GemmProblem p = gemm(dhb, (size_t)Mq * D, D, Wo, (size_t)D * Da, Da, Mq, Da, D, EPI_BF16, c_.dctx, Da);
        TRY(launch_gemm(&p, 1, GEMM_NN, -1, st));
    }
    if (tail) TRY(launch_attn_bwd_win(a.qkv, a.ctx, c_.dctx, a.lse, c_.delta, dqkv, B, N, s.H, s.hdp, tail->nvis, tail->ndec, st, sm_scale));
    else TRY(launch_attn_bwd(a.qkv, a.ctx, c_.dctx, a.lse, c_.delta, dqkv, B, N, s.H, s.hdp, st, sm_scale));
    if (fuse) {
        GemmProblem p = gemm(dqkv, (size_t)M * 3 * Da, 3 * Da, Wqkv, (size_t)3 * Da * D, D, M, D, 3 * Da, EPI_DLN, dres, D);
        p.C2 = dyb_next; p.ln_x = x_in; p.ln_mean = a.mean1; p.ln_rstd = a.rstd1; p.ln_gamma = P + o.ln1w;
        p.ln_part = c_.ln_part; p.ln_dgamma = G + o.ln1w; p.ln_dbeta = G + o.ln1b;
        TRY(launch_gemm(&p, 1, GEMM_NN, -1, st));
    } else {
        GemmProblem p = gemm(dqkv, (size_t)M * 3 * Da, 3 * Da, Wqkv, (size_t)3 * Da * D, D, M, D, 3 * Da, EPI_BF16, c_.dln, D);
        TRY(launch_gemm(&p, 1, GEMM_NN, -1, st));
    }
    hipStream_t ws = st;
    if (c_.overlap) {
        BVC_CHECK_HIP(hipEventRecord(c_.ev_fork, st));
        BVC_CHECK_HIP(hipStreamWaitEvent(c_.side, c_.ev_fork, 0));
        ws = c_.side;
    }
    {
        GemmProblem g[4];
        g[0] = gemm(dyb, (size_t)Mq * D, D, a.act, (size_t)Mq * I, I, D, I, Mq, EPI_F32, G + o.w2, I);
        g[1] = gemm(dh, (size_t)Mq * I, I, a.ln2o, (size_t)Mq * D, D, I, D, Mq, EPI_F32, G + o.w1, D);
        g[2] = gemm(dhb, (size_t)Mq * D, D, a.ctx, (size_t)Mq * Da, Da, D, Da, Mq, EPI_F32, pad ? s.gwo_pad : G + o.wo, Da);
        g[3] = gemm(dqkv, (size_t)M * 3 * Da, 3 * Da, a.ln1o, (size_t)M * D, D, 3 * Da, D, M, EPI_F32, pad ? s.gwqkv_pad : G + o.wqkv, D);
        g[0].rowsum = G + o.b2;
        g[1].rowsum = G + o.b1;
        g[2].rowsum = G + o.bo;
        g[3].rowsum = pad ? s.gbqkv_pad : G + o.bqkv;
        const int tile = plan_dw(g, 4);
        if (pad) {
            BVC_CHECK_HIP(hipMemsetAsync(s.gwo_pad, 0, (size_t)D * Da * 4, ws));
            BVC_CHECK_HIP(hipMemsetAsync(s.gwqkv_pad, 0, (size_t)3 * Da * D * 4, ws));
            BVC_CHECK_HIP(hipMemsetAsync(s.gbqkv_pad, 0, (size_t)3 * Da * 4, ws));
        }
        TRY(launch_gemm(g, 4, GEMM_TN, tile, ws));
        if (pad)
            TRY(launch_unpad_head_grads(s.gwqkv_pad, s.gbqkv_pad, s.gwo_pad, G + o.wqkv, G + o.bqkv, G + o.wo, D, s.H, s.hd, s.hdp, ws));
    }
    if (!fuse) TRY(launch_ln_bwd(c_.dln, x_in, identity_rows(), a.mean1, a.rstd1, P + o.ln1w, dres, 1, dyb_next, G + o.ln1w, G + o.ln1b, c_.ln_part, M, D, st,
                                 gated && li > 0 ? &g_below : nullptr));
    if (c_.overlap) {
// ... 13 lines not shown
```

baby-vision-curriculum_amd/csrc/videomae.hip:

```cpp
#include <math.h>
#include <stdarg.h>
#include <stdio.h>
#include <stdlib.h>
#include <string.h>

#include <algorithm>
#include <string>
#include <vector>

#include "stack.h"

namespace bvc {
static thread_local char g_err[1024] = "";
void set_error(const char* fmt, ...) {
    va_list ap;
    va_start(ap, fmt);
    vsnprintf(g_err, sizeof(g_err), fmt, ap);
    va_end(ap);
}
const char* last_error() { return g_err; }
}

using namespace bvc;

// ... 43 lines not shown
    L.head_w = L.add("decoder.head.weight", {P, Dd});
    L.head_b = L.add("decoder.head.bias", {P});
    return L;
}

}

struct bvc_ctx {
    bvc_videomae_config cfg;
    Layout lay;
    int max_batch, nmask, nvis, L, P, Kp;
    int ndec, Ld;
    Arena arena;
    Work w;
    float *pos_enc, *pos_dec;
    int batch = 0;
    bool have_forward = false;
    bf16_t* wbf;
    bool shadow_valid = false;
    const float* params = nullptr;
    int *vis_idx, *dec_idx, *status;
    bf16_t* Ape;
    Stack enc, dec;
    bf16_t* xe_bf;
    float *meanf, *rstdf;
    bf16_t* lnf;
    float* labels;
    bf16_t* diff;
    float* partial;
    int npartial = 0;
    float *dres_enc, *dres_dec;
    bf16_t* de2d;
    bool tail_on = false;
};

namespace {

void sinusoid(std::vector<float>& out, int n, int d) {
    out.resize((size_t)n * d);
    for (int p = 0; p < n; ++p)
        for (int j = 0; j < d; ++j) {
            const double ang = (double)p / pow(10000.0, 2.0 * (j / 2) / (double)d);
            out[(size_t)p * d + j] = (float)((j & 1) ? cos(ang) : sin(ang));
        }
}

}

namespace {
int pixel_src(const void* pixels, const bvc_pixel_format* fmt, int channels, PixelSrc* out) {
    PixelSrc px = pixels_f32((const float*)pixels);
    if (fmt && fmt->dtype != BVC_PIXELS_F32) {
        BVC_REQUIRE(fmt->dtype == BVC_PIXELS_U8, "pixel format: dtype %d unknown", fmt->dtype);
        BVC_REQUIRE(channels <= 4, "pixel format: uint8 input supports at most 4 channels");
        px.is_u8 = 1;
        for (int c = 0; c < 4; ++c) {
            BVC_REQUIRE(fmt->std[c] != 0.f || c >= channels, "pixel format: std[%d] is zero", c);
            px.mean[c] = fmt->mean[c];
            px.stdv[c] = c < channels ? fmt->std[c] : 1.f;
        }
    }
    *out = px;
    return BVC_OK;
}
}

extern "C" {

const char* bvc_last_error(void) { return bvc::last_error(); }
const char* bvc_version(void) { return "gfx950;bvc-hip-r5"; }

int bvc_set_option(const char* name, int value) {
    BVC_REQUIRE(name != nullptr, "set_option: null name");
    if (!strcmp(name, "gemm8")) { BVC_REQUIRE(value >= -1 && value <= 1, "set_option: gemm8 takes -1 / 0 / 1"); options().gemm8 = value; }
    else if (!strcmp(name, "dw_overlap")) options().dw_overlap = value != 0;
    else if (!strcmp(name, "row_stagger")) options().row_stagger = value != 0;
    else if (!strcmp(name, "row_ln")) { BVC_REQUIRE(value >= -1 && value <= 1, "set_option: row_ln takes -1 / 0 / 1"); options().row_ln = value; }
    else if (!strcmp(name, "deterministic")) { BVC_REQUIRE(value == 0 || value == 1, "set_option: deterministic takes 0 / 1"); options().deterministic = value; }
    else if (!strcmp(name, "head_pad")) { BVC_REQUIRE(value == 0 || value == 1, "set_option: head_pad takes 0 / 1"); options().head_pad = value; }
    else if (!strcmp(name, "dec_tail")) { BVC_REQUIRE(value == 0 || value == 1, "set_option: dec_tail takes 0 / 1"); options().dec_tail = value; }
    else BVC_REQUIRE(false, "set_option: unknown option '%s'", name);
    return BVC_OK;
}
int bvc_get_option(const char* name) {
    if (name && !strcmp(name, "gemm8")) return options().gemm8;
    if (name && !strcmp(name, "dw_overlap")) return options().dw_overlap;
    if (name && !strcmp(name, "row_ln")) return options().row_ln;
    if (name && !strcmp(name, "row_stagger")) return options().row_stagger;
    if (name && !strcmp(name, "deterministic")) return options().deterministic;
    if (name && !strcmp(name, "head_pad")) return options().head_pad;
    if (name && !strcmp(name, "dec_tail")) return options().dec_tail;
    bvc::set_error("get_option: unknown option '%s'", name ? name : "(null)");
    return BVC_ERR_INVALID;
}

int bvc_videomae_param_count(const bvc_videomae_config* cfg) {
    if (!cfg || check_config(*cfg) != BVC_OK) return BVC_ERR_INVALID;
    return (int)make_layout(*cfg).entries.size();
}

int64_t bvc_videomae_param_numel(const bvc_videomae_config* cfg) {
    if (!cfg || check_config(*cfg) != BVC_OK) return BVC_ERR_INVALID;
    return make_layout(*cfg).total;
}

int bvc_videomae_param_info(const bvc_videomae_config* cfg, int index, char* name, int name_cap, int64_t* offset,
                            int64_t* numel, int* ndim, int64_t shape[5]) {
    BVC_REQUIRE(cfg && name && offset && numel && ndim && shape, "param_info: null argument");
    TRY(check_config(*cfg));
    const Layout L = make_layout(*cfg);
    BVC_REQUIRE(index >= 0 && index < (int)L.entries.size(), "param_info: index %d out of range", index);
    const ParamEntry& e = L.entries[index];
    snprintf(name, name_cap, "%s", e.name.c_str());
    *offset = e.offset; *numel = e.numel; *ndim = e.ndim;
    for (int i = 0; i < 5; ++i) shape[i] = e.shape[i];
    return BVC_OK;
}

void bvc_videomae_destroy(bvc_ctx* c) {
    if (!c) return;
    free_work(c->w);
    c->arena.release();
    delete c;
}
// ... 31 lines not shown
    const size_t B = max_batch, Mv = B * c->nvis, Md = B * c->Ld, Mm = B * c->ndec;
    const int D = cfg->hidden_size, Dd = cfg->decoder_hidden_size, I = cfg->intermediate_size, Id = cfg->decoder_intermediate_size;
    const int H = cfg->num_attention_heads, Hd = cfg->decoder_num_attention_heads;
    int rc = BVC_OK;
    auto fail = [&](int r) { bvc_videomae_destroy(c); return r; };
    {
        const size_t we = std::max<size_t>(3 * (size_t)H * attn_width(D / H), (size_t)I), wd = std::max<size_t>(3 * (size_t)Hd * attn_width(Dd / Hd), (size_t)Id);
        const size_t ee = Mv * we * 2, ed = Md * wd * 2;
        if (ee >= 0xFFFFFFF0ull || ed >= 0xFFFFFFF0ull) {
            const bool dec = ed >= ee;
            set_error("create: max_batch %d exceeds the 4 GiB operand extent: the %s's %zu tokens x %zu bf16 columns are %.2f GiB; at most %zu clips",
                      max_batch, dec ? "decoder" : "encoder", dec ? Md : Mv, dec ? wd : we, (dec ? ed : ee) / 1073741824.0,
                      (size_t)(0xFFFFFFEFull / std::max((dec ? ed : ee) / B, (size_t)1)));
            delete c;
            return BVC_ERR_INVALID;
        }
    }
#define A(expr) if ((rc = (expr)) != BVC_OK) return fail(rc)
    A(c->arena.alloc(&c->pos_enc, (size_t)c->L * D));
    A(c->arena.alloc(&c->pos_dec, (size_t)c->L * Dd));
    A(c->arena.alloc(&c->wbf, (size_t)c->lay.total));
    A(c->arena.alloc(&c->vis_idx, Mv));
    A(c->arena.alloc(&c->dec_idx, Mm));
    if (hipMemset(c->vis_idx, 0, (size_t)Mv * sizeof(int)) != hipSuccess || hipMemset(c->dec_idx, 0, (size_t)Mm * sizeof(int)) != hipSuccess) {
        set_error("videomae_create: hipMemset of the token lists failed");
        bvc_videomae_destroy(c);
        return BVC_ERR_HIP;
    }
    A(c->arena.alloc(&c->status, 4));
    A(c->arena.alloc(&c->Ape, Mv * c->Kp));
    A(alloc_stack(c->arena, c->enc, D, I, H, cfg->num_hidden_layers, cfg->layer_norm_eps, Mv, B * H * c->nvis));
    A(alloc_stack(c->arena, c->dec, Dd, Id, Hd, cfg->decoder_num_hidden_layers, cfg->layer_norm_eps, Md, B * Hd * c->Ld));
    A(c->arena.alloc(&c->xe_bf, Mv * D));
    A(c->arena.alloc(&c->meanf, Mm));
    A(c->arena.alloc(&c->rstdf, Mm));
    A(c->arena.alloc(&c->lnf, Mm * Dd));
    A(c->arena.alloc(&c->labels, Mm * c->P));
    A(c->arena.alloc(&c->diff, Mm * c->P));
    A(c->arena.alloc(&c->partial, (Mm / 64 + 2) * (c->P / 64 + 2)));
    A(c->arena.alloc(&c->dres_enc, Mv * D));
    A(c->arena.alloc(&c->dres_dec, Md * Dd));
    const size_t MD = std::max(Mv * D, Md * Dd), MI = std::max(Mv * I, Md * Id);
    A(c->arena.alloc(&c->de2d, Mv * Dd));
    A(alloc_work(c->arena, c->w, MD, MI, std::max(B * H * c->nvis, B * Hd * c->Ld),
                 std::max(ln_bwd_workspace_floats_upto((int)Mv, D), ln_bwd_workspace_floats_upto((int)Md, Dd))));
#undef A
    std::vector<float> tab;
    sinusoid(tab, c->L, D);
    if (hipMemcpy(c->pos_enc, tab.data(), tab.size() * 4, hipMemcpyHostToDevice) != hipSuccess) { set_error("create: pos upload failed"); return fail(BVC_ERR_HIP); }
    sinusoid(tab, c->L, Dd);
    if (hipMemcpy(c->pos_dec, tab.data(), tab.size() * 4, hipMemcpyHostToDevice) != hipSuccess) { set_error("create: pos upload failed"); return fail(BVC_ERR_HIP); }
    *out = c;
    return BVC_OK;
}

int bvc_videomae_forward(bvc_ctx* c, const float* pixels, const uint8_t* mask, int batch, const float* params,
                         float* loss, float* logits, void* stream) {
    return bvc_videomae_forward_px(c, pixels, nullptr, mask, batch, params, loss, logits, stream);
}

int bvc_videomae_forward_px(bvc_ctx* c, const void* pixels_any, const bvc_pixel_format* fmt, const uint8_t* mask, int batch,
                            const float* params, float* loss, float* logits, void* stream) {
    return bvc_videomae_forward_dual(c, pixels_any, fmt, mask, nullptr, batch, params, loss, logits, stream);
}

int bvc_videomae_forward_dual(bvc_ctx* c, const void* pixels_any, const bvc_pixel_format* fmt, const uint8_t* mask, const uint8_t* decode_mask,
// ... 11 lines not shown
    const int D = cf.hidden_size, Dd = cf.decoder_hidden_size, P = c->P;
    c->have_forward = false;
    c->batch = B;
    c->params = params;
    c->w.params = params;
    c->w.wbf = c->wbf;
    const PatchGeom pg{cf.num_frames, cf.num_channels, cf.image_size, cf.image_size, cf.tubelet_size, cf.patch_size};

    if (!c->shadow_valid) TRY(launch_cast_bf16(params, c->wbf, (size_t)L.total, st));
    c->shadow_valid = false;
    BVC_CHECK_HIP(hipMemsetAsync(c->status, 0, 16, st));
    if (decode_mask) TRY(launch_dual_mask_index(mask, decode_mask, B, Lq, nvis, ndec, c->vis_idx, c->dec_idx, c->status, st));
    else TRY(launch_mask_index(mask, B, Lq, nvis, ndec, c->vis_idx, c->dec_idx, c->status, st));
    TRY(launch_gather_patches(pixels, c->vis_idx, c->Ape, B, nvis, pg, st));
    {
        GemmProblem p = gemm(c->Ape, (size_t)Mv * c->Kp, c->Kp, c->wbf + L.pe_w, (size_t)D * c->Kp, c->Kp, Mv, D, c->Kp, EPI_POS,
                             c->enc.act[0].x_in, D);
        p.bias = params + L.pe_b; p.rowtok = c->vis_idx; p.pos = c->pos_enc;
        TRY(launch_gemm(&p, 1, GEMM_NT, -1, st));
    }
    for (int i = 0; i < c->enc.nlayers; ++i) {
        float* xo = i + 1 < c->enc.nlayers ? c->enc.act[i + 1].x_in : c->enc.x_out;
        TRY(layer_forward(c->w, c->enc, i, L.enc[i], c->enc.act[i].x_in, xo, B, nvis, st, i + 1 < c->enc.nlayers ? &L.enc[i + 1] : nullptr));
    }
    TRY(launch_gather_rows_bf16(c->enc.x_out, identity_rows(), c->xe_bf, Mv, D, st));
    {
        GemmProblem p = gemm(c->xe_bf, (size_t)Mv * D, D, c->wbf + L.e2d_w, (size_t)Dd * D, D, Mv, Dd, D, EPI_E2D, c->dec.act[0].x_in, Dd);
        p.rowtok = c->vis_idx; p.pos = c->pos_dec; p.rin = nvis; p.rout = Ld;
        TRY(launch_gemm(&p, 1, GEMM_NT, -1, st));
    }
    TRY(launch_fill_masked(c->dec.act[0].x_in, params + L.mask_token, c->pos_dec, c->dec_idx, B, Ld, nvis, ndec, Dd, st));
    const LayerTail lt{nvis, ndec};
    c->tail_on = layer_tail_ok(c->w, c->dec, B, nvis, ndec);
    for (int i = 0; i < c->dec.nlayers; ++i) {
        const bool last = i + 1 == c->dec.nlayers;
        float* xo = !last ? c->dec.act[i + 1].x_in : c->dec.x_out;
        TRY(layer_forward(c->w, c->dec, i, L.dec[i], c->dec.act[i].x_in, xo, B, Ld, st, !last ? &L.dec[i + 1] : nullptr, last && c->tail_on ? &lt : nullptr));
    }
    const RowMap tail = c->tail_on ? identity_rows() : RowMap{ndec, Ld, nvis};
    TRY(launch_ln_fwd(c->dec.x_out, tail, params + L.norm_w, params + L.norm_b, c->lnf, c->meanf, c->rstdf, Mm, Dd, cf.decoder_norm_eps, st));
    TRY(launch_labels(pixels, c->dec_idx, c->labels, B, ndec, pg, cf.norm_pix_loss, st));
    {
        GemmProblem p = gemm(c->lnf, (size_t)Mm * Dd, Dd, c->wbf + L.head_w, (size_t)P * Dd, Dd, Mm, P, Dd, EPI_LOSS, c->diff, P);
        p.bias = params + L.head_b; p.labels = c->labels; p.partial = c->partial; p.C2 = logits;
        c->npartial = gemm_num_tiles(p, -1);
        TRY(launch_gemm(&p, 1, GEMM_NT, -1, st));
    }
    TRY(launch_loss_finalize(c->partial, c->npartial, (double)Mm * (double)P, c->status, loss, st));
    c->have_forward = true;
    return BVC_OK;
}

int bvc_videomae_backward(bvc_ctx* c, const float* grad_loss, float* G, bvc_bucket_fn on_bucket, void* user, void* stream) {
    BVC_REQUIRE(c && grad_loss && G, "backward: null argument");
    if (!c->have_forward) { set_error("backward: no forward state (call bvc_videomae_forward first; one backward per forward)"); return BVC_ERR_STATE; }
    c->have_forward = false;
    hipStream_t st = (hipStream_t)stream;
    const bvc_videomae_config& cf = c->cfg;
    const Layout& L = c->lay;
    const int B = c->batch, nvis = c->nvis, ndec = c->ndec, Ld = c->Ld;
    const int Mv = B * nvis, Md = B * Ld, Mm = B * ndec;
    const int D = cf.hidden_size, Dd = cf.decoder_hidden_size, P = c->P;
    const bf16_t* W = c->wbf;
    const float* params = c->params;
    auto bucket = [&](int64_t lo, int64_t hi) { if (on_bucket) on_bucket(lo, hi - lo, user); };
    begin_backward(c->w);

    BVC_CHECK_HIP(hipMemsetAsync(G, 0, (size_t)L.total * 4, st));
    const float cmse = (float)(2.0 / ((double)Mm * (double)P));
    {
        GemmProblem p = gemm(c->diff, (size_t)Mm * P, P, c->lnf, (size_t)Mm * Dd, Dd, P, Dd, Mm, EPI_F32, G + L.head_w, Dd);
        p.alpha = cmse; p.alpha_dev = grad_loss;
        p.rowsum = G + L.head_b;
        const int tile = plan_dw(&p, 1);
        TRY(launch_gemm(&p, 1, GEMM_TN, tile, st));
    }
    {
        GemmProblem p = gemm(c->diff, (size_t)Mm * P, P, W + L.head_w, (size_t)P * Dd, Dd, Mm, Dd, P, EPI_BF16, c->w.dln, Dd);
        p.alpha = cmse; p.alpha_dev = grad_loss;
        TRY(launch_gemm(&p, 1, GEMM_NN, -1, st));
    }
    const RowMap tail{ndec, Ld, nvis};
    const LayerTail lt{nvis, ndec};
    if (c->tail_on) {
        BVC_CHECK_HIP(hipMemset2DAsync(c->dres_dec, (size_t)Ld * Dd * 4, 0, (size_t)nvis * Dd * 4, (size_t)B, st));
        TRY(launch_ln_bwd(c->w.dln, c->dec.x_out, tail, c->meanf, c->rstdf, params + L.norm_w, c->dres_dec, 0, c->w.dyb[0],
                          G + L.norm_w, G + L.norm_b, c->w.ln_part, Mm, Dd, st, nullptr, true));
    } else {
        BVC_CHECK_HIP(hipMemsetAsync(c->dres_dec, 0, (size_t)Md * Dd * 4, st));
        BVC_CHECK_HIP(hipMemsetAsync(c->w.dyb[0], 0, (size_t)Md * Dd * 2, st));
        TRY(launch_ln_bwd(c->w.dln, c->dec.x_out, tail, c->meanf, c->rstdf, params + L.norm_w, c->dres_dec, 0, c->w.dyb[0],
                          G + L.norm_w, G + L.norm_b, c->w.ln_part, Mm, Dd, st));
    }
    bucket(L.norm_w, L.total);
    for (int i = c->dec.nlayers - 1; i >= 0; --i) {
        TRY(layer_backward(c->w, c->dec, i, L.dec[i], c->dec.act[i].x_in, c->dres_dec, G, B, Ld, st, on_bucket, user,
                           i + 1 == c->dec.nlayers && c->tail_on ? &lt : nullptr));
    }
    TRY(launch_colsum_f32(c->dres_dec, tail, Mm, Dd, G + L.mask_token, st));
    const RowMap headrows{nvis, Ld, 0};
    TRY(launch_gather_rows_bf16(c->dres_dec, headrows, c->de2d, Mv, Dd, st));
    {
        GemmProblem p = gemm(c->de2d, (size_t)Mv * Dd, Dd, c->xe_bf, (size_t)Mv * D, D, Dd, D, Mv, EPI_F32, G + L.e2d_w, D);
        const int tile = plan_dw(&p, 1);
        TRY(launch_gemm(&p, 1, GEMM_TN, tile, st));
    }
    {
        GemmProblem p = gemm(c->de2d, (size_t)Mv * Dd, Dd, W + L.e2d_w, (size_t)Dd * D, D, Mv, D, Dd, EPI_F32_BF16, c->dres_enc, D);
        p.C2 = c->w.dyb[c->w.seq % 3];
        TRY(launch_gemm(&p, 1, GEMM_NN, -1, st));
    }
    bucket(L.e2d_w, L.dec.front().ln1w);
    for (int i = c->enc.nlayers - 1; i >= 0; --i) {
        TRY(layer_backward(c->w, c->enc, i, L.enc[i], c->enc.act[i].x_in, c->dres_enc, G, B, nvis, st, on_bucket, user));
    }
    {
        GemmProblem p = gemm(c->w.dyb[c->w.seq % 3], (size_t)Mv * D, D, c->Ape, (size_t)Mv * c->Kp, c->Kp, D, c->Kp, Mv, EPI_F32, G + L.pe_w, c->Kp);
        p.rowsum = G + L.pe_b;
        const int tile = plan_dw(&p, 1);
        TRY(launch_gemm(&p, 1, GEMM_TN, tile, st));
    }
    TRY(join_side(c->w, c->w.seq & 1, st, on_bucket, user));
    TRY(join_side(c->w, (c->w.seq + 1) & 1, st, on_bucket, user));
    bucket(0, L.enc.front().ln1w);
    return BVC_OK;
}

static int tail_tap(bvc_ctx* c, float* dst, hipStream_t st) {
    const Layout& L = c->lay;
    Stack& s = c->dec;
    LayerAct& a = s.act.back();
    const LayerOff& o = L.dec.back();
// ... 483 lines not shown
int bvc_op_colsum_f32(const float* X, int rin, int rout, int roff, int M, int D, float* out, void* stream) {
    BVC_REQUIRE(X && out && M > 0 && D > 0, "op_colsum_f32: bad argument");
    return launch_colsum_f32(X, RowMap{rin, rout, roff}, M, D, out, (hipStream_t)stream);
}
int bvc_op_colsum_bf16(const void* X, int M, int N, int ld, float alpha, const float* alpha_dev, float* out, void* stream) {
    BVC_REQUIRE(X && out, "op_colsum_bf16: null argument");
    return launch_colsum_bf16_scaled((const bf16_t*)X, M, N, ld, alpha, alpha_dev, out, (hipStream_t)stream);
}
int bvc_op_sgd_step(float* params, float* grads, float* momentum_buf, int64_t n, float lr, float momentum, float dampening,
                    float weight_decay, int nesterov, int first_step, int maximize, const float* grad_scale,
                    const float* found_inf, int write_unscaled_grads, void* bf16_shadow, void* stream) {
    BVC_REQUIRE(params && grads && n >= 0, "op_sgd_step: bad argument");
    return launch_sgd_step(params, grads, momentum_buf, (size_t)n, lr, momentum, dampening, weight_decay, nesterov, first_step,
                           maximize, grad_scale, found_inf, write_unscaled_grads, (bf16_t*)bf16_shadow, (hipStream_t)stream);
}
int bvc_op_adam_prepare(float* state3, double lr, double beta1, double beta2, const float* found_inf, void* stream) {
    BVC_REQUIRE(state3, "op_adam_prepare: null state");
    return launch_adam_prep(state3, lr, beta1, beta2, found_inf, (hipStream_t)stream);
}
int bvc_op_adam_step(float* params, float* grads, float* exp_avg, float* exp_avg_sq, int64_t n, double lr, double beta1, double beta2,
                     double eps, double weight_decay, int decoupled, int maximize, const float* state3, const float* grad_scale,
                     const float* found_inf, int write_unscaled_grads, void* bf16_shadow, void* stream) {
    BVC_REQUIRE(params && grads && exp_avg && exp_avg_sq && state3 && n >= 0, "op_adam_step: bad argument");
    return launch_adam_step(params, grads, exp_avg, exp_avg_sq, (size_t)n, lr, beta1, beta2, eps, weight_decay, decoupled, maximize,
                            state3, grad_scale, found_inf, write_unscaled_grads, (bf16_t*)bf16_shadow, (hipStream_t)stream);
}
int bvc_op_row_ln_selected(int tokens, int width, int mlp_width, int heads) {
    if (tokens <= 0 || width <= 0 || heads <= 0 || width % heads != 0) return 0;
    Stack s;
    s.D = width; s.I = mlp_width; s.H = heads; s.nlayers = 0; s.eps = 0.f; s.x_out = nullptr;
    s.hd = width / heads; s.hdp = attn_width(s.hd); s.Da = heads * s.hdp;
    return fuse_row_ln(s, tokens) ? 1 : 0;
}
int bvc_op_sgd_step_segments(float* params, float* grads, float* momentum_buf, int64_t n, const int64_t* seg_start, const int32_t* seg_group,
                             const int32_t* blk_seg, int nseg, const bvc_sgd_groups* groups, const float* grad_scale, const float* found_inf,
                             int write_unscaled_grads, void* bf16_shadow, void* stream) {
    BVC_REQUIRE(params && grads && n >= 0, "op_sgd_step_segments: bad argument");
    return launch_sgd_step_segments(params, grads, momentum_buf, n, seg_start, seg_group, blk_seg, nseg, groups, grad_scale, found_inf,
                                    write_unscaled_grads, (bf16_t*)bf16_shadow, (hipStream_t)stream);
}
int bvc_op_adam_step_segments(float* params, float* grads, float* exp_avg, float* exp_avg_sq, int64_t n, const int64_t* seg_start,
                              const int32_t* seg_group, const int32_t* blk_seg, int nseg, const bvc_adam_groups* groups, float* state,
                              double* hyper_scratch, const float* grad_scale, const float* found_inf, int write_unscaled_grads,
                              void* bf16_shadow, void* stream) {
    BVC_REQUIRE(params && grads && exp_avg && exp_avg_sq && n >= 0, "op_adam_step_segments: bad argument");
    return launch_adam_step_segments(params, grads, exp_avg, exp_avg_sq, n, seg_start, seg_group, blk_seg, nseg, groups, state, hyper_scratch,
                                     grad_scale, found_inf, write_unscaled_grads, (bf16_t*)bf16_shadow, (hipStream_t)stream);
}
int bvc_videomae_shadow(bvc_ctx* c, int valid, void** shadow_bf16, int64_t* numel) {
    BVC_REQUIRE(c, "videomae_shadow: null context");
    if (shadow_bf16) *shadow_bf16 = c->wbf;
    if (numel) *numel = (int64_t)c->lay.total;
    if (valid >= 0) c->shadow_valid = valid != 0;
    return BVC_OK;
}
int bvc_op_nonfinite_check(const float* x, int64_t n, float* found_inf, void* stream) {
    BVC_REQUIRE(x && found_inf && n >= 0, "op_nonfinite_check: bad argument");
    return launch_nonfinite_check(x, (size_t)n, found_inf, (hipStream_t)stream);
}
int bvc_op_row_normalize(const float* f, void* fn_bf16, float* inv_norm, int n, int p, float eps, void* stream) {
    BVC_REQUIRE(f && fn_bf16 && inv_norm, "op_row_normalize: null argument");
    return launch_row_normalize(f, (bf16_t*)fn_bf16, inv_norm, n, p, eps, (hipStream_t)stream);
}
int bvc_op_row_normalize_bwd(const float* f, const float* inv_norm, const float* dfn, float* df, int n, int p, void* stream) {
    BVC_REQUIRE(f && inv_norm && dfn && df, "op_row_normalize_bwd: null argument");
    return launch_row_normalize_bwd(f, inv_norm, dfn, df, n, p, (hipStream_t)stream);
// ... 32 lines not shown
```

baby-vision-curriculum_amd/probe.py:

```python
import ctypes

import torch

from . import _lib, _ops

PEAK_BF16_TFLOPS = 2500.0
PEAK_HBM_GBS = 8000.0


def _time(fn, iters=5, warm=2):
    for _ in range(warm):
        fn()
    e0, e1 = torch.cuda.Event(enable_timing=True), torch.cuda.Event(enable_timing=True)
    e0.record()
    for _ in range(iters):
        fn()
    e1.record()
    torch.cuda.synchronize()
    return e0.elapsed_time(e1) * 1e3 / iters


def _rb(dev, *shape):
    return torch.randn(*shape, device=dev, dtype=torch.bfloat16)


def _gemm_rows(dev, B, add):
    E = _ops.EPI
    Mv, Md, Mm = B * 160, B * 1568, B * 1408
    D, I, Dd, Id, P = 768, 3072, 384, 1536, 1536

    def one(label, layout, M, N, K, epi, count, tile=-1):
        A = _rb(dev, M, K)
        Bm = _rb(dev, N, K) if layout == _ops.NT else _rb(dev, K, N)
        Bm.mul_(0.02)
        kw = {}
        out_f32 = epi in ("F32", "RESID", "POS", "E2D", "F32_BF16", "RESID_LN", "DLN")
        nbytes = 2.0 * (M * K + N * K)
        Mo = M
        if epi == "E2D":
            Mo = (M // 160) * 1568
        C = torch.empty(Mo, N, device=dev, dtype=torch.float32 if out_f32 else torch.bfloat16)
        nbytes += (4.0 if out_f32 else 2.0) * M * N
        if epi not in ("DGELU", "E2D", "DLN"):
            kw["bias"] = torch.zeros(N, device=dev)
        if epi == "GELU":
            kw["C2"] = torch.empty_like(C)
            nbytes += 2.0 * M * N
        if epi == "F32_BF16":
            kw["C2"] = torch.empty(M, N, device=dev, dtype=torch.bfloat16)
            nbytes += 2.0 * M * N
        if epi in ("RESID", "RESID_LN"):
            kw["resid"] = torch.randn(M, N, device=dev)
            nbytes += 4.0 * M * N
        if epi == "RESID_LN":
            kw.update(C2=torch.empty(M, N, device=dev, dtype=torch.bfloat16), ln_gamma=torch.ones(N, device=dev), ln_beta=torch.zeros(N, device=dev),
                      ln_mean=torch.empty(M, device=dev), ln_rstd=torch.empty(M, device=dev), ln_eps=1e-12)
            nbytes += 2.0 * M * N
        if epi == "DLN":
            kw.update(C2=torch.empty(M, N, device=dev, dtype=torch.bfloat16), ln_gamma=torch.ones(N, device=dev), ln_x=torch.randn(M, N, device=dev),
                      ln_mean=torch.zeros(M, device=dev), ln_rstd=torch.ones(M, device=dev), ln_part=torch.empty(512 * 2 * N, device=dev),
                      ln_dgamma=torch.zeros(N, device=dev), ln_dbeta=torch.zeros(N, device=dev))
            nbytes += (4.0 + 4.0 + 2.0) * M * N
        if epi == "DGELU":
            kw["aux"] = _rb(dev, M, N)
            nbytes += 2.0 * M * N
        if epi in ("POS", "E2D"):
            kw["rowtok"] = (torch.arange(M, device=dev, dtype=torch.int32) % 160) * 9
            kw["pos"] = torch.randn(1568, N, device=dev)
            nbytes += 4.0 * M * N
            if epi == "E2D":
                kw["rin"], kw["rout"] = 160, 1568
        if epi == "LOSS":
            kw["labels"] = torch.randn(M, N, device=dev)
            kw["partial"] = torch.empty(1 << 16, device=dev)
            nbytes += 4.0 * M * N
        d = _ops.gemm_desc(A, Bm, M, N, K, E[epi], C, **kw)
        name = _ops.gemm_kernel_name(d, layout, tile)
        us = _time(lambda: _ops.gemm(d, layout, tile))
        add(name, label, count, us, 2.0 * M * N * K, nbytes)

    def dw_single(label, Mo, No, K, count):
        A, Bm = _rb(dev, K, Mo), _rb(dev, K, No)
        C = torch.zeros(Mo, No, device=dev)
        rs = torch.zeros(Mo, device=dev)
        d = _ops.gemm_desc(A, Bm, Mo, No, K, E["F32"], C, rowsum=rs)
        tile, _ = _ops.plan_dw([d])
        name = _ops.gemm_kernel_name(d, _ops.TN, tile)
        us = _time(lambda: _ops.gemm(d, _ops.TN, tile))
        add(name, label, count, us, 2.0 * Mo * No * K, 2.0 * K * (Mo + No) + 4.0 * Mo * No)

    def dw_group(label, M, Dm, Im, count):
        dy, act, dh, ln2, dqkv = _rb(dev, M, Dm), _rb(dev, M, Im), _rb(dev, M, Im), _rb(dev, M, Dm), _rb(dev, M, 3 * Dm)
        shapes = [(Dm, Im), (Im, Dm), (Dm, Dm), (3 * Dm, Dm)]
        outs = [torch.zeros(s, device=dev) for s in shapes]
        bs = [torch.zeros(s[0], device=dev) for s in shapes]
        ds = [_ops.gemm_desc(dy, act, Dm, Im, M, E["F32"], outs[0], rowsum=bs[0]),
              _ops.gemm_desc(dh, ln2, Im, Dm, M, E["F32"], outs[1], rowsum=bs[1]),
              _ops.gemm_desc(dy, ln2, Dm, Dm, M, E["F32"], outs[2], rowsum=bs[2]),
              _ops.gemm_desc(dqkv, ln2, 3 * Dm, Dm, M, E["F32"], outs[3], rowsum=bs[3])]
        tile, split = _ops.plan_dw(ds)
        name = _ops.gemm_kernel_name(ds, _ops.TN, tile)
        us = _time(lambda: _ops.gemm(ds, _ops.TN, tile), iters=3)
        fl = 2.0 * M * (2 * Dm * Im + 4 * Dm * Dm)
        nb = 2.0 * M * (2 * Dm + 2 * Im + 2 * Dm + Dm + 3 * Dm) + 4.0 * (2 * Dm * Im + 4 * Dm * Dm)
        add(name, f"{label} (tile {tile}, split {split})", count, us, fl, nb)

    NT, NN = _ops.NT, _ops.NN
    fused = bool(_lib.lib().bvc_op_row_ln_selected(Md, Dd, Id, 6))
    one("patch embed", NT, Mv, D, 1536, "POS", 1)
    one("enc qkv", NT, Mv, 3 * D, D, "BF16", 12)
    one("enc proj", NT, Mv, D, D, "RESID", 12)
    one("enc fc1+GELU", NT, Mv, I, D, "GELU", 12)
    one("enc fc2", NT, Mv, D, I, "RESID", 12)
    one("enc->dec", NT, Mv, Dd, D, "E2D", 1)
    one("dec qkv", NT, Md, 3 * Dd, Dd, "BF16", 4)
    if fused:
        one("dec proj + LayerNorm", NT, Md, Dd, Dd, "RESID_LN", 4)
    else:
        one("dec proj", NT, Md, Dd, Dd, "RESID", 4)
    one("dec fc1+GELU", NT, Md, Id, Dd, "GELU", 4)
    if fused:
        one("dec fc2 + next LayerNorm", NT, Md, Dd, Id, "RESID_LN", 3)
        one("dec fc2", NT, Md, Dd, Id, "RESID", 1)
    else:
        one("dec fc2", NT, Md, Dd, Id, "RESID", 4)
    one("head+MSE", NT, Mm, P, Dd, "LOSS", 1)
    one("head dX", NN, Mm, Dd, P, "BF16", 1)
    one("dec dX fc2", NN, Md, Id, Dd, "DGELU", 4)
    one("dec dX fc1 + LayerNorm bwd" if fused else "dec dX fc1", NN, Md, Dd, Id, "DLN" if fused else "BF16", 4)
    one("dec dX proj", NN, Md, Dd, Dd, "BF16", 4)
    one("dec dX qkv + LayerNorm bwd" if fused else "dec dX qkv", NN, Md, Dd, 3 * Dd, "DLN" if fused else "BF16", 4)
    one("enc->dec dX", NN, Mv, D, Dd, "F32_BF16", 1)
    one("enc dX fc2", NN, Mv, I, D, "DGELU", 12)
    one("enc dX fc1", NN, Mv, D, I, "BF16", 12)
    one("enc dX proj", NN, Mv, D, D, "BF16", 12)
    one("enc dX qkv", NN, Mv, D, 3 * D, "BF16", 12)
    dw_single("head dW", P, Dd, Mm, 1)
    dw_single("enc->dec dW", Dd, D, Mv, 1)
    dw_single("patch dW", D, 1536, Mv, 1)
    dw_group("dec layer dW group", Md, Dd, Id, 4)
    dw_group("enc layer dW group", Mv, D, I, 12)


def _attention_rows(dev, B, add):
    lib = _lib.lib()
    st = _lib.current_stream_ptr
    for label, N, H, count in (("enc", 160, 12, 12), ("dec", 1568, 6, 4)):
        Dm = 64 * H
        qkv, ctx, dctx, dqkv = _rb(dev, B * N, 3 * Dm), _rb(dev, B * N, Dm), _rb(dev, B * N, Dm), _rb(dev, B * N, 3 * Dm)
        lse = torch.empty(B * H * N, device=dev)
        delta = torch.empty(B * H * N, device=dev)
        p = lambda t: ctypes.c_void_p(t.data_ptr())
        fwd = lambda: _lib.check(lib.bvc_op_attention_fwd(p(qkv), p(ctx), p(lse), B, N, H, 64, st()), "attention_fwd")
        dq = lambda: _lib.check(lib.bvc_op_attention_bwd_part(p(qkv), p(ctx), p(dctx), p(lse), p(delta), p(dqkv), B, N, H, 64, 1, st()), "attention_bwd dq")
        dkv = lambda: _lib.check(lib.bvc_op_attention_bwd_part(p(qkv), p(ctx), p(dctx), p(lse), p(delta), p(dqkv), B, N, H, 64, 2, st()), "attention_bwd dkdv")
        unit = 2.0 * N * N * 64 * H * B
        tok = 2.0 * B * N * Dm
        add("bvc::attn_fwd_kernel<64>", f"{label} attention fwd", count, _time(fwd), 2 * unit, 4 * tok)
        if N <= 160:
            bwd = lambda: _lib.check(lib.bvc_op_attention_bwd(p(qkv), p(ctx), p(dctx), p(lse), p(delta), p(dqkv), B, N, H, 64, st()), "attention_bwd")
            add(f"bvc::attn_bwd_head_kernel<64, {5 if N > 128 else 0}>", f"{label} attention bwd (whole head: S, dP, dV, dK, dQ)", count, _time(bwd),
                5 * unit, 8 * tok)
            continue
        add("bvc::attn_bwd_dq_kernel<64>", f"{label} attention bwd dQ (S, dP, dQ)", count, _time(dq), 3 * unit, 6 * tok)
        add("bvc::attn_bwd_dkdv_kernel<64>", f"{label} attention bwd dK dV (recomputes S, dP)", count, _time(dkv), 2 * unit, 6 * tok)


def _layernorm_rows(dev, B, add):
    lib = _lib.lib()
    st = _lib.current_stream_ptr
    p = lambda t: ctypes.c_void_p(t.data_ptr())
    fused = bool(lib.bvc_op_row_ln_selected(B * 1568, 384, 1536, 6))
    for label, M, Dm, count, count_bwd in (("enc", B * 160, 768, 24, 24), ("dec", B * 1568, 384, 1 if fused else 8, 0 if fused else 8),
                                           ("final", B * 1408, 384, 1, 1)):
        x, dres = torch.randn(M, Dm, device=dev), torch.randn(M, Dm, device=dev)
        gmm, bta = torch.ones(Dm, device=dev), torch.zeros(Dm, device=dev)
        y, dy, dresb = _rb(dev, M, Dm), _rb(dev, M, Dm), _rb(dev, M, Dm)
        mean, rstd = torch.empty(M, device=dev), torch.empty(M, device=dev)
        dg, db = torch.zeros(Dm, device=dev), torch.zeros(Dm, device=dev)
        ws = torch.empty(int(lib.bvc_op_layernorm_bwd_workspace(M, Dm)), device=dev)
        fwd = lambda: _lib.check(lib.bvc_op_layernorm_fwd(p(x), 0, 0, 0, p(gmm), p(bta), p(y), p(mean), p(rstd), M, Dm, 1e-12, st()), "layernorm_fwd")
        bwd = lambda: _lib.check(lib.bvc_op_layernorm_bwd(p(dy), p(x), 0, 0, 0, p(mean), p(rstd), p(gmm), p(dres), 1, p(dresb), p(dg), p(db),
                                                          p(ws), M, Dm, st()), "layernorm_bwd")
        e = float(M) * Dm
        add("bvc::ln_fwd_kernel", f"{label} LayerNorm fwd", count, _time(fwd), 0.0, 6 * e)
        if count_bwd:
            add("bvc::ln_bwd_kernel (+ ln_param_reduce)", f"{label} LayerNorm bwd", count_bwd, _time(bwd), 0.0, 16 * e)


def step_kernels(batch, device):
    rows = {}

    def add(kernel, label, count, us, flops, nbytes):
        r = rows.setdefault(kernel, {"kernel": kernel, "launches_per_step": 0, "us_per_step": 0.0, "flops": 0.0, "bytes": 0.0, "products": []})
        r["launches_per_step"] += count
        r["us_per_step"] += count * us
        r["flops"] += count * flops
        r["bytes"] += count * nbytes
        r["products"].append({"name": label, "launches": count, "launch_us": round(us, 1),
                              "tflops": round(flops / us / 1e6, 1), "gb_per_s": round(nbytes / us / 1e3, 1)})

    with torch.no_grad():
        _gemm_rows(device, batch, add)
        _attention_rows(device, batch, add)
        _layernorm_rows(device, batch, add)
    torch.cuda.empty_cache()
# ... 15 lines not shown
```

include/bvc.h:

```cpp
#ifndef BVC_H
#define BVC_H

#include <stddef.h>
#include <stdint.h>

#ifdef __cplusplus
extern "C" {
#endif

#define BVC_OK 0
#define BVC_ERR_INVALID (-1)
#define BVC_ERR_HIP (-2)
#define BVC_ERR_STATE (-3)

const char* bvc_last_error(void);
const char* bvc_version(void);
int bvc_set_option(const char* name, int value);
int bvc_get_option(const char* name);
int64_t bvc_deterministic_workspace_bytes(void);
int bvc_deterministic_workspace_release(void);

typedef struct bvc_videomae_config {
    int image_size, patch_size, num_channels, num_frames, tubelet_size;
    int hidden_size, num_hidden_layers, num_attention_heads, intermediate_size;
// ... 129 lines not shown
int bvc_op_token_mean(const float* x, int batch, int ntok, int dim, float* out, void* stream);
int bvc_op_token_mean_bwd(const float* dmean, int batch, int ntok, int dim, float* dx, void* stream);

enum { BVC_GEMM_NT = 0, BVC_GEMM_NN = 1, BVC_GEMM_TN = 2 };
enum {
    BVC_EPI_F32 = 0, BVC_EPI_BF16 = 1, BVC_EPI_GELU = 2, BVC_EPI_RESID = 3, BVC_EPI_POS = 4, BVC_EPI_E2D = 5,
    BVC_EPI_LOSS = 6, BVC_EPI_DGELU = 7, BVC_EPI_F32_BF16 = 8, BVC_EPI_RELU = 9, BVC_EPI_DRELU = 10,
    BVC_EPI_NCE = 11, BVC_EPI_NCE_BWD = 12, BVC_EPI_RESID_LN = 13, BVC_EPI_DLN = 14, BVC_EPI_RESID_GATE = 15
};
typedef struct bvc_gemm_desc {
    const void* A; const void* B;
    int M, N, K, lda, ldb;
    uint32_t a_bytes, b_bytes;
    float alpha;
    const float* alpha_dev;
    int epi, split_k;
    void* C; int ldc; int seg_rows; void* C2;
    const float* bias; const float* resid; const void* aux; int ldaux; int seg_stride;
    const int* rowtok; const float* pos; const float* labels; float* partial;
    int rin, rout;
    float* rowsum;
    const float* ln_gamma; const float* ln_beta;
    float* ln_mean; float* ln_rstd;
    float ln_eps; int seg_off;
    const float* ln_x;
    float* ln_part; float* ln_dgamma; float* ln_dbeta;
} bvc_gemm_desc;
int bvc_op_gemm(const bvc_gemm_desc* problems, int count, int layout, int tile_cfg, int stages, void* stream);
int bvc_op_gemm_num_tiles(const bvc_gemm_desc* problem, int tile_cfg);
int bvc_op_gemm_gate(const bvc_gemm_desc* problem, const bvc_branch_drop* drop, int layer, int branch, int tile_cfg, void* stream);
int bvc_op_gemm_gate_kernel(const bvc_gemm_desc* problem, int tile_cfg, char* name, int name_cap);
int bvc_op_gemm_kernel(const bvc_gemm_desc* problems, int count, int layout, int tile_cfg, int stages, char* name, int name_cap);
int bvc_op_row_ln_selected(int tokens, int width, int mlp_width, int heads);
int bvc_op_gemm_plan_dw(bvc_gemm_desc* problems, int count);

int bvc_op_attention_fwd(const void* qkv, void* ctx_out, float* lse, int B, int N, int H, int head_dim, void* stream);
int bvc_op_attention_bwd(const void* qkv, const void* ctx_in, const void* dctx, const float* lse, float* delta_scratch,
                         void* dqkv, int B, int N, int H, int head_dim, void* stream);
int bvc_op_attention_bwd_part(const void* qkv, const void* ctx_in, const void* dctx, const float* lse, float* delta_scratch,
                              void* dqkv, int B, int N, int H, int head_dim, int part, void* stream);
int bvc_op_attention_width(int head_dim);
int bvc_op_attention_fwd_scaled(const void* qkv, void* ctx_out, float* lse, int B, int N, int H, int head_dim, float softmax_scale,
                                void* stream);
int bvc_op_attention_bwd_scaled(const void* qkv, const void* ctx_in, const void* dctx, const float* lse, float* delta_scratch,
                                void* dqkv, int B, int N, int H, int head_dim, float softmax_scale, void* stream);
int bvc_op_attention_probs(const void* qkv, const float* lse, float* probs, int B, int N, int H, int head_dim, float softmax_scale,
                           void* stream);
int bvc_op_layernorm_fwd(const float* x, int rin, int rout, int roff, const float* gamma, const float* beta, void* y_bf16,
                         float* mean, float* rstd, int M, int D, float eps, void* stream);
int bvc_op_layernorm_bwd(const void* dy_bf16, const float* x, int rin, int rout, int roff, const float* mean,
                         const float* rstd, const float* gamma, float* dres, int accumulate, void* dres_bf16,
                         float* dgamma, float* dbeta, float* workspace, int M, int D, void* stream);
int64_t bvc_op_layernorm_bwd_workspace(int M, int D);
int bvc_op_layernorm_bwd_gate(const void* dy_bf16, const float* x, const float* mean, const float* rstd, const float* gamma, float* dres,
                              int accumulate, void* dres_bf16, float* dgamma, float* dbeta, float* workspace, int M, int D,
                              const bvc_branch_drop* drop, int layer, int branch, void* stream);
int bvc_op_colsum_bf16(const void* X, int M, int N, int ld, float alpha, const float* alpha_dev, float* out, void* stream);
int bvc_op_colsum_f32(const float* X, int rin, int rout, int roff, int M, int D, float* out, void* stream);
int bvc_op_cast_bf16(const float* in, void* out, int64_t n, void* stream);
int bvc_op_row_normalize(const float* f, void* fn_bf16, float* inv_norm, int n, int p, float eps, void* stream);
int bvc_op_row_normalize_bwd(const float* f, const float* inv_norm, const float* dfn, float* df, int n, int p, void* stream);
int bvc_op_nce_finalize(const float* partial, int ntiles, float inv_temperature, int64_t npos, float* loss, float* stats, void* stream);
int bvc_op_sgd_step(float* params, float* grads, float* momentum_buf, int64_t n, float lr, float momentum, float dampening,
                    float weight_decay, int nesterov, int first_step, int maximize, const float* grad_scale,
                    const float* found_inf, int write_unscaled_grads, void* bf16_shadow, void* stream);
int bvc_op_adam_prepare(float* state3, double lr, double beta1, double beta2, const float* found_inf, void* stream);
// ... 50 lines not shown
```

Measured before the change: 3276 clips/s.

## Compute decoder layer-0 LN/QKV for masked tokens once from a shared position table

In the first decoder layer, masked-token rows are all mask_token+pos embedding, so their LayerNorm and QKV projection depend only on position. The change computes LN and QKV once for a per-position table plus the visible rows, then assembles the full per-clip tensors by gather. In backward, a new DLN epilogue variant (EC 7) skips stores for tiles made only of decoded rows and accumulates their column sums for the mask-token gradient, and the colsum skips those rows. This cuts GEMM and LayerNorm work on roughly 90% of decoder layer-0 rows, at the cost of extra kernels, scratch buffers and considerable complexity.

```diff
diff --git a/baby-vision-curriculum_amd/_lib.py b/baby-vision-curriculum_amd/_lib.py
--- a/baby-vision-curriculum_amd/_lib.py
+++ b/baby-vision-curriculum_amd/_lib.py
@@ -216,6 +216,7 @@
     "bvc_op_adam_step": (c_int, [c_void_p, c_void_p, c_void_p, c_void_p, c_int64, c_double, c_double, c_double, c_double, c_double,
                                  c_int, c_int, c_void_p, c_void_p, c_void_p, c_int, c_void_p, c_void_p]),
     "bvc_op_row_ln_selected": (c_int, [c_int, c_int, c_int, c_int]),
+    "bvc_op_dec_head_selected": (c_int, [c_int, c_int, c_int, c_int, c_int, c_int, c_int]),
     "bvc_op_sgd_step_segments": (c_int, [c_void_p, c_void_p, c_void_p, c_int64, c_void_p, c_void_p, c_void_p, c_int, c_void_p, c_void_p, c_void_p,
                                          c_int, c_void_p, c_void_p]),
     "bvc_op_adam_step_segments": (c_int, [c_void_p, c_void_p, c_void_p, c_void_p, c_int64, c_void_p, c_void_p, c_void_p, c_int, c_void_p, c_void_p,
diff --git a/baby-vision-curriculum_amd/csrc/gemm.h b/baby-vision-curriculum_amd/csrc/gemm.h
--- a/baby-vision-curriculum_amd/csrc/gemm.h
+++ b/baby-vision-curriculum_amd/csrc/gemm.h
@@ -30,7 +30,7 @@
 
 constexpr int kMaxGroup = 4;
 
-struct Options { int gemm8 = 0; int dw_overlap = 0; int row_ln = 0; int row_stagger = 1; int deterministic = 0; int head_pad = 0; int dec_tail = 1; };
+struct Options { int gemm8 = 0; int dw_overlap = 0; int row_ln = 0; int row_stagger = 1; int deterministic = 0; int head_pad = 0; int dec_tail = 1; int dec_head = 1; };
 Options& options();
 
 float* det_scratch(size_t floats, hipStream_t stream);
@@ -48,5 +48,7 @@
 int gemm_pick_tile(const GemmProblem* probs, int nprob, int tile_cfg);
 bool gemm_row_ln_ok(int M, int N, int K);
 constexpr size_t kRowLnPartFloats = 512 * 2 * 384;
+constexpr int kRowLnSkipRows = 512;
+constexpr size_t kRowLnSkipFloats = (size_t)kRowLnSkipRows * 384;
 
 }
diff --git a/baby-vision-curriculum_amd/csrc/gemm.hip b/baby-vision-curriculum_amd/csrc/gemm.hip
--- a/baby-vision-curriculum_amd/csrc/gemm.hip
+++ b/baby-vision-curriculum_amd/csrc/gemm.hip
@@ -354,6 +354,9 @@
         BVC_REQUIRE(p.C && p.C2 && p.ln_mean && p.ln_rstd && p.ln_gamma, "launch_gemm: LayerNorm epilogue with a null output / statistic / scale");
         if (p.epi == EPI_RESID_LN) BVC_REQUIRE(layout == GEMM_NT && p.resid && p.ln_beta, "launch_gemm: RESID_LN is an NT product with a residual and a LayerNorm bias");
         if (p.epi == EPI_DLN) BVC_REQUIRE(layout == GEMM_NN && p.ln_x && p.ln_part && p.ln_dgamma && p.ln_dbeta, "launch_gemm: DLN is an NN product with the LayerNorm input, partial scratch and parameter gradients");
+        if (p.epi == EPI_DLN && p.rout != 0)
+            BVC_REQUIRE(p.rin >= 0 && p.rout > p.rin && p.M % p.rout == 0 && p.partial != nullptr && p.seg_rows == 0,
+                        "launch_gemm: bad skip map (rin %d, rout %d: clips of rout rows that divide M = %d, partial scratch, no segment map)", p.rin, p.rout, p.M);
         if (p.seg_rows != 0)
             BVC_REQUIRE(p.seg_rows > 0 && p.seg_rows % 128 == 0 && p.M % p.seg_rows == 0 && p.seg_off >= 0 && p.seg_stride > 0 &&
                             (long long)p.seg_off + p.seg_rows <= (long long)p.seg_stride,
diff --git a/baby-vision-curriculum_amd/csrc/gemm8.hip b/baby-vision-curriculum_amd/csrc/gemm8.hip
--- a/baby-vision-curriculum_amd/csrc/gemm8.hip
+++ b/baby-vision-curriculum_amd/csrc/gemm8.hip
@@ -95,8 +95,8 @@
     extern __shared__ __attribute__((aligned(16))) char smem[];
     static_assert(BM == 256 || (BM == 128 && BN == 384), "128-row tiles: the 128 x 384 geometry only");
     static_assert(BN == 256 || BN == 128 || (BN == 384 && BM == 128), "column tiles of 256 / 128, or 384 with 128 rows");
-    static_assert((EC == 4 || EC == 5) == (BM == 128 && !AT), "row epilogues (EC 4 / 5) are the k-contiguous-A instantiations of the 128 x 384 tile, and only they");
-    static_assert(BM == 256 || EC == 4 || EC == 5 || (AT && BT && (EC == 2 || EC == 6)), "128 x 384 with transposed A: weight gradients");
+    static_assert((EC == 4 || EC == 5 || EC == 7) == (BM == 128 && !AT), "row epilogues (EC 4 / 5 / 7) are the k-contiguous-A instantiations of the 128 x 384 tile, and only they");
+    static_assert(BM == 256 || EC == 4 || EC == 5 || EC == 7 || (AT && BT && (EC == 2 || EC == 6)), "128 x 384 with transposed A: weight gradients");
     static_assert(EC != 6 || (AT && BT), "EC 6 (deterministic weight gradients) is a TN product");
     static_assert(EC != 4 || !BT, "EC 4 (residual + LayerNorm forward) is an NT product");
     constexpr int A_BYTES = BM * 64 * 2, B_BYTES = BN * 64 * 2, TILE = A_BYTES + B_BYTES;
@@ -112,7 +112,9 @@
 #else
     constexpr bool LATE = false;
 #endif
-    constexpr int PAR_BYTES = EC == 4 ? 3 * BN * 4 : EC == 5 ? BN * 4 : 0, STAT_OFF = PAR_BYTES, COL_OFF = STAT_OFF + 4096;
+    constexpr bool DLN = EC == 5 || EC == 7;
+    constexpr int NACC = EC == 7 ? 3 : 2;
+    constexpr int PAR_BYTES = EC == 4 ? 3 * BN * 4 : DLN ? BN * 4 : 0, STAT_OFF = PAR_BYTES, COL_OFF = STAT_OFF + 4096;
     constexpr int CPR = BN == 384 ? 8 : WN / 8;
     constexpr int NSIDE = TM * (16 / (64 / CPR));
     static_assert(PT + 2 * NSIDE < 64, "vmcnt is a 6-bit counter");
@@ -140,13 +142,17 @@
         }
     }
     if (uid >= u_hi) {
-        if constexpr (EC == 5) {
+        if constexpr (DLN) {
             float* pr = g.prob[0].ln_part + (size_t)blockIdx.x * 2 * BN;
             for (int i = tid; i < 2 * BN; i += 512) pr[i] = 0.f;
         }
+        if constexpr (EC == 7) {
+            float* pr = g.prob[0].partial + (size_t)blockIdx.x * BN;
+            for (int i = tid; i < BN; i += 512) pr[i] = 0.f;
+        }
         return;
     }
-    if constexpr (EC == 4 || EC == 5) {
+    if constexpr (EC == 4 || DLN) {
         const int cnt = x_hi - x_lo, r = cnt % nslots, nmax = (cnt + nslots - 1) / nslots;
         int num = 0, den = 1;
         if (r > 0 && slot_id >= r) { num = slot_id - r + 1; den = nslots - r + 1; }
@@ -270,7 +276,7 @@
         for (int i = tid; i < npad; i += 512) lbias[i] = (p0.bias && i < p0.N) ? p0.bias[i] : 0.f;
         __syncthreads();
     }
-    if constexpr (EC == 4 || EC == 5) {
+    if constexpr (EC == 4 || DLN) {
         const GemmProblem& p0 = g.prob[0];
         AS3 float* lpar = (AS3 float*)((AS3 char*)smem + 2 * TILE);
         for (int i = tid; i < BN; i += 512) {
@@ -282,9 +288,9 @@
                 lpar[i] = p0.ln_gamma[i];
             }
         }
-        if constexpr (EC == 5) {
+        if constexpr (DLN) {
             AS3 float* lcol = (AS3 float*)((AS3 char*)smem + 2 * TILE + COL_OFF);
-            for (int i = tid; i < 8 * 2 * WN; i += 512) lcol[i] = 0.f;
+            for (int i = tid; i < 8 * NACC * WN; i += 512) lcol[i] = 0.f;
         }
         __syncthreads();
     }
@@ -446,7 +452,7 @@
         const int m0 = cu.m0, n0 = cu.n0;
         const int epi = p.epi, Mrows = p.M, Ncols = p.N, ldc = p.ldc;
         int seg_shift = 0;
-        if constexpr (EC == 4 || EC == 5) {
+        if constexpr (EC == 4 || DLN) {
             if (p.seg_rows > 0) {
                 const int upc = p.seg_rows >> 7, u = m0 >> 7, c = u / upc;
                 seg_shift = __builtin_amdgcn_readfirstlane(c * p.seg_stride + p.seg_off + ((u - c * upc) << 7) - m0);
@@ -598,13 +604,18 @@
                     __builtin_amdgcn_raw_buffer_store_b128(u32x4{s0[0], s1[0], s0[1], s1[1]}, rc2, o2 + 64u * jp, 0, BVC_G8_ROW_ST_AUX);
                 }
             }
-        } else if constexpr (EC == 5) {
+        } else if constexpr (DLN) {
             const uint32_t ext = (uint32_t)Mrows * (uint32_t)(BN * 4);
             const __amdgpu_buffer_rsrc_t rx = make_rsrc(p.ln_x, ext), rd = make_rsrc(reinterpret_cast<float*>(p.C) + (size_t)seg_shift * BN, ext), rc2 = make_rsrc(p.C2, ext / 2);
             const __amdgpu_buffer_rsrc_t rmu = make_rsrc(p.ln_mean, (uint32_t)Mrows * 4u), rrs = make_rsrc(p.ln_rstd, (uint32_t)Mrows * 4u);
             const AS3 float* lpar = (const AS3 float*)((AS3 char*)smem + 2 * TILE);
             AS3 float* lstat = (AS3 float*)((AS3 char*)smem + 2 * TILE + STAT_OFF);
-            AS3 float* lcol = (AS3 float*)((AS3 char*)smem + 2 * TILE + COL_OFF) + wave * 2 * WN;
+            AS3 float* lcol = (AS3 float*)((AS3 char*)smem + 2 * TILE + COL_OFF) + wave * NACC * WN;
+            bool skip_unit = false;
+            if constexpr (EC == 7) {
+                const int jr = m0 % p.rout;
+                skip_unit = __builtin_amdgcn_readfirstlane((jr >= p.rin && jr + BM <= p.rout) ? 1 : 0) != 0;
+            }
             const int q4 = lane >> 4, r16 = lane & 15;
             const int cw = wn * WN + 4 * q4;
             const int mrow = m0 + 16 * wm + r16;
@@ -665,7 +676,26 @@
 #pragma unroll
                 for (int j = 0; j < TN; ++j) {
                     acc[i][j] = ((acc[i][j] - c1) - xr[b][j] * c2) * rsd[b] + dr[j];
-                    __builtin_amdgcn_raw_buffer_store_b128(__builtin_bit_cast(u32x4, acc[i][j]), rd, obase + (uint32_t)(i * 32 * BN * 4 + 64 * j), 0, BVC_G8_ROW_ST_AUX);
+                    if constexpr (EC != 7)
+                        __builtin_amdgcn_raw_buffer_store_b128(__builtin_bit_cast(u32x4, acc[i][j]), rd, obase + (uint32_t)(i * 32 * BN * 4 + 64 * j), 0, BVC_G8_ROW_ST_AUX);
+                }
+                if constexpr (EC == 7) {
+                    if (skip_unit) {
+#pragma unroll
+                        for (int j = 0; j < TN; ++j) {
+                            f32x4 td = acc[i][j];
+#pragma unroll
+                            for (int e = 0; e < 4; ++e) td[e] = row16_sum(td[e]);
+                            if (r16 == 0) {
+                                AS3 f32x4* cd = reinterpret_cast<AS3 f32x4*>(lcol + 2 * WN + 16 * j + 4 * q4);
+                                *cd = *cd + td;
+                            }
+                        }
+                        return;
+                    }
+#pragma unroll
+                    for (int j = 0; j < TN; ++j)
+                        __builtin_amdgcn_raw_buffer_store_b128(__builtin_bit_cast(u32x4, acc[i][j]), rd, obase + (uint32_t)(i * 32 * BN * 4 + 64 * j), 0, BVC_G8_ROW_ST_AUX);
                 }
 #pragma unroll
                 for (int jp = 0; jp < TN / 2; ++jp) {
@@ -886,19 +916,26 @@
         uid += u_step;
         if (uid >= u_hi) break;
         decode_unit<BM, BN>(g, uid, cu);
-        after_epi = (EC == 4 || EC == 5) ? -1 : (((EC == 2 || EC == 6) && atomic) || BN == 384) ? 0 : EC == 0 ? nstores : -1;
+        after_epi = (EC == 4 || DLN) ? -1 : (((EC == 2 || EC == 6) && atomic) || BN == 384) ? 0 : EC == 0 ? nstores : -1;
     }
     wait_vmcnt<0>();
 #ifndef BVC_G8_NO_STAGGER
     if (wm == 0) asm volatile("s_barrier" ::: "memory");
 #endif
-    if constexpr (EC == 5) {
+    if constexpr (DLN) {
         __syncthreads();
         const AS3 float* lcol = (const AS3 float*)((AS3 char*)smem + 2 * TILE + COL_OFF);
         float* pr = g.prob[0].ln_part + (size_t)blockIdx.x * 2 * BN;
         for (int c = tid; c < 2 * BN; c += 512) {
             const int which = c / BN, col = c % BN, w = col / WN, cc = col % WN;
-            pr[c] = lcol[(w * 2 + which) * WN + cc] + lcol[((4 + w) * 2 + which) * WN + cc];
+            pr[c] = lcol[(w * NACC + which) * WN + cc] + lcol[((4 + w) * NACC + which) * WN + cc];
+        }
+        if constexpr (EC == 7) {
+            float* pd = g.prob[0].partial + (size_t)blockIdx.x * BN;
+            for (int c = tid; c < BN; c += 512) {
+                const int w = c / WN, cc = c % WN;
+                pd[c] = lcol[(w * NACC + 2) * WN + cc] + lcol[((4 + w) * NACC + 2) * WN + cc];
+            }
         }
     }
 }
@@ -942,7 +979,7 @@
 
 template <int BM, int BN, bool AT, bool BT, int EC>
 static int launch_gemm8_one(const GemmGroup& g_in, int total, hipStream_t stream) {
-    constexpr size_t lds = 2 * (size_t)(BM + BN) * 64 * 2 + (EC == 0 ? (size_t)32768 : EC == 4 ? (size_t)(3 * BN * 4 + 4096) : EC == 5 ? (size_t)(BN * 4 + 4096 + 8 * 2 * (BN / 4) * 4) :
+    constexpr size_t lds = 2 * (size_t)(BM + BN) * 64 * 2 + (EC == 0 ? (size_t)32768 : EC == 4 ? (size_t)(3 * BN * 4 + 4096) : EC == 5 ? (size_t)(BN * 4 + 4096 + 8 * 2 * (BN / 4) * 4) : EC == 7 ? (size_t)(BN * 4 + 4096 + 8 * 3 * (BN / 4) * 4) :
                                                               BN == 384 ? (size_t)8 * 16 * 48 * 4 : (size_t)8 * 16 * (BN / 4) * 4);
     static_assert(lds <= 160 * 1024, "LDS per CU");
     if (dry_run().on) {
@@ -961,14 +998,14 @@
     if constexpr (EC == 2) {
         if (plan_balance(g, BM, BN, total, ncu)) grid = ncu;
     }
-    if constexpr (EC == 4 || EC == 5) {
+    if constexpr (EC == 4 || EC == 5 || EC == 7) {
         const double us = 1.45 * ((g.prob[0].K + 63) / 64) + (EC == 4 ? 23.0 : 32.0);
         g.stagger = options().row_stagger && total > ncu ? (int)(us * 33.0) : 0;
     }
     hipLaunchKernelGGL((gemm8_kernel<BM, BN, AT, BT, EC>), dim3(grid), dim3(512), lds, stream, g, total);
     BVC_CHECK_HIP(hipGetLastError());
     (void)0;
-    if constexpr (EC == 5)
+    if constexpr (EC == 5 || EC == 7)
         return launch_ln_param_reduce(g.prob[0].ln_part, grid, BN, g.prob[0].ln_dgamma, g.prob[0].ln_dbeta, stream);
     return BVC_OK;
 }
@@ -1007,7 +1044,8 @@
         const GemmProblem& p = g.prob[0];
         if (g.nprob != 1 || p.N != 384 || p.ldc != 384 || (double)p.M * 1536.0 >= 4294000000.0) return 1;
         if (ec == 4 && layout == GEMM_NT) return launch_gemm8_one<128, 384, false, false, 4>(g, total, stream);
-        if (ec == 5 && layout == GEMM_NN) return launch_gemm8_one<128, 384, false, true, 5>(g, total, stream);
+        if (ec == 5 && layout == GEMM_NN) return p.rout > 0 ? launch_gemm8_one<128, 384, false, true, 7>(g, total, stream)
+                                                            : launch_gemm8_one<128, 384, false, true, 5>(g, total, stream);
         return 1;
     }
     if (ec >= 4) return 1;
diff --git a/baby-vision-curriculum_amd/csrc/rowops.h b/baby-vision-curriculum_amd/csrc/rowops.h
--- a/baby-vision-curriculum_amd/csrc/rowops.h
+++ b/baby-vision-curriculum_amd/csrc/rowops.h
@@ -27,7 +27,7 @@
 int launch_ln_param_reduce(const float* part, int nblk, int D, float* dgamma, float* dbeta, hipStream_t s);
 int launch_colsum_bf16(const bf16_t* X, int M, int N, int ld, float alpha, float* out, hipStream_t s);
 int launch_colsum_bf16_scaled(const bf16_t* X, int M, int N, int ld, float alpha, const float* alpha_dev, float* out, hipStream_t s);
-int launch_colsum_f32(const float* X, RowMap rm, int M, int D, float* out, hipStream_t s);
+int launch_colsum_f32(const float* X, RowMap rm, int M, int D, float* out, hipStream_t s, int skip_nvis = 0, int skip_ld = 0);
 int launch_token_mean(const float* x, int B, int N, int D, float* out, hipStream_t s);
 int launch_token_mean_bwd(const float* dmean, int B, int N, int D, float* dx, hipStream_t s);
 int launch_fcnorm_bwd_bcast(const float* dy, const float* p, const float* mean, const float* rstd, const float* gamma, float* dres,
@@ -43,6 +43,8 @@
 int launch_labels(PixelSrc clip, const int* dec_idx, float* labels, int B, int ndec, PatchGeom pg, int norm_pix, hipStream_t s);
 int launch_fill_masked(float* xfull, const float* mask_token, const float* pos, const int* dec_idx, int B, int Ld, int nvis,
                        int ndec, int D, hipStream_t s);
+int launch_head_assemble(const bf16_t* ln_s, const bf16_t* qkv_s, const float* mean_s, const float* rstd_s, const int* dec_idx, bf16_t* ln1o,
+                         bf16_t* qkv, float* mean1, float* rstd1, int B, int L, int Ld, int nvis, int D, int Q, hipStream_t s);
 int launch_sgd_step(float* p, float* g, float* buf, size_t n, float lr, float momentum, float dampening, float wd, int nesterov,
                     int first, int maximize, const float* grad_scale, const float* found_inf, int write_grad, bf16_t* shadow,
                     hipStream_t s);
diff --git a/baby-vision-curriculum_amd/csrc/rowops.hip b/baby-vision-curriculum_amd/csrc/rowops.hip
--- a/baby-vision-curriculum_amd/csrc/rowops.hip
+++ b/baby-vision-curriculum_amd/csrc/rowops.hip
@@ -287,15 +287,22 @@
 }
 
 template <bool DET>
-__device__ __forceinline__ void colsum_f32_body(const float* __restrict__ X, RowMap rm, int M, int D, float* __restrict__ out, int RB) {
+__device__ __forceinline__ void colsum_f32_body(const float* __restrict__ X, RowMap rm, int M, int D, float* __restrict__ out, int RB,
+                                                int skip_nvis, int skip_ld) {
     __shared__ float red[4][256];
     const int lane = threadIdx.x & 63, wave = threadIdx.x >> 6;
     const int col = (blockIdx.x * 64 + lane) * 4;
     f32x4 acc = {0, 0, 0, 0};
     const int r0 = blockIdx.y * RB, r1 = min(M, r0 + RB);
     if (col < D)
-        for (int m = r0 + wave; m < r1; m += 4)
-            acc += *reinterpret_cast<const f32x4*>(X + (size_t)map_row(m, rm) * D + col);
+        for (int m = r0 + wave; m < r1; m += 4) {
+            const int pr = map_row(m, rm);
+            if (skip_ld > 0) {
+                const int jr = (pr & ~127) % skip_ld;
+                if (jr >= skip_nvis && jr + 128 <= skip_ld) continue;
+            }
+            acc += *reinterpret_cast<const f32x4*>(X + (size_t)pr * D + col);
+        }
 #pragma unroll
     for (int e = 0; e < 4; ++e) red[wave][lane * 4 + e] = acc[e];
     __syncthreads();
@@ -308,12 +315,12 @@
     }
 }
 __global__ __launch_bounds__(256) void colsum_f32_kernel(const float* __restrict__ X, RowMap rm, int M, int D,
-                                                         float* __restrict__ out, int RB) {
-    colsum_f32_body<false>(X, rm, M, D, out, RB);
+                                                         float* __restrict__ out, int RB, int skip_nvis, int skip_ld) {
+    colsum_f32_body<false>(X, rm, M, D, out, RB, skip_nvis, skip_ld);
 }
 __global__ __launch_bounds__(256) void colsum_f32_det_kernel(const float* __restrict__ X, RowMap rm, int M, int D,
-                                                             float* __restrict__ part, int RB) {
-    colsum_f32_body<true>(X, rm, M, D, part, RB);
+                                                             float* __restrict__ part, int RB, int skip_nvis, int skip_ld) {
+    colsum_f32_body<true>(X, rm, M, D, part, RB, skip_nvis, skip_ld);
 }
 
 __global__ __launch_bounds__(256) void token_mean_kernel(const float* __restrict__ x, int N, int D, float* __restrict__ out) {
@@ -712,6 +719,46 @@
     const f32x4 mt = reinterpret_cast<const f32x4*>(mask_token)[c];
     const f32x4 pe = reinterpret_cast<const f32x4*>(pos + (size_t)dec_idx[m] * D)[c];
     reinterpret_cast<f32x4*>(xfull + ((size_t)b * Ld + nvis + j) * D)[c] = mt + pe;
+}
+
+template <int CL, int CQ>
+__global__ __launch_bounds__(256) void head_assemble_kernel(const bf16_t* __restrict__ ln_s, const bf16_t* __restrict__ qkv_s,
+                                                            const float* __restrict__ mean_s, const float* __restrict__ rstd_s,
+                                                            const int* __restrict__ dec_idx, bf16_t* __restrict__ ln1o,
+                                                            bf16_t* __restrict__ qkv, float* __restrict__ mean1, float* __restrict__ rstd1,
+                                                            int B, int L, int Ld, int nvis, int D, int Q) {
+    const int lane = threadIdx.x & 63, wave = threadIdx.x >> 6;
+    const int nl = D >> 3, nq = Q >> 3, ndec = Ld - nvis;
+    const int run = blockIdx.x & 7, slot = blockIdx.x >> 3, nslots = gridDim.x >> 3;
+    const int lo = (int)((long long)Ld * run / 8), len = (int)((long long)Ld * (run + 1) / 8) - lo;
+    const int items = B * len;
+    for (int t = slot * 4 + wave; t < items; t += nslots * 4) {
+        const int b = t / len, j = lo + (t - b * len);
+        const int r = b * Ld + j;
+        const int src = j < nvis ? L + b * nvis + j : dec_idx[b * ndec + (j - nvis)];
+        const f32x4* sl = reinterpret_cast<const f32x4*>(ln_s + (size_t)src * D);
+        const f32x4* sq = reinterpret_cast<const f32x4*>(qkv_s + (size_t)src * Q);
+        f32x4* dl = reinterpret_cast<f32x4*>(ln1o + (size_t)r * D);
+        f32x4* dq = reinterpret_cast<f32x4*>(qkv + (size_t)r * Q);
+        if constexpr (CL > 0) {
+            f32x4 vl[CL], vq[CQ];
+#pragma unroll
+            for (int i = 0; i < CL; ++i) vl[i] = sl[min(lane + 64 * i, nl - 1)];
+#pragma unroll
+            for (int i = 0; i < CQ; ++i) vq[i] = sq[min(lane + 64 * i, nq - 1)];
+#pragma unroll
+            for (int i = 0; i < CL; ++i) if (lane + 64 * i < nl) dl[lane + 64 * i] = vl[i];
+#pragma unroll
+            for (int i = 0; i < CQ; ++i) if (lane + 64 * i < nq) dq[lane + 64 * i] = vq[i];
+        } else {
+            for (int c = lane; c < nl; c += 64) dl[c] = sl[c];
+            for (int c = lane; c < nq; c += 64) dq[c] = sq[c];
+        }
+        if (lane == 0) {
+            mean1[r] = mean_s[src];
+            rstd1[r] = rstd_s[src];
+        }
+    }
 }
 
 __global__ __launch_bounds__(256) void loss_finalize_kernel(const float* __restrict__ partial, int n, double count,
@@ -1301,19 +1348,20 @@
     return launch_colsum_bf16_scaled(X, M, N, ld, alpha, nullptr, out, s);
 }
 
-int launch_colsum_f32(const float* X, RowMap rm, int M, int D, float* out, hipStream_t s) {
+int launch_colsum_f32(const float* X, RowMap rm, int M, int D, float* out, hipStream_t s, int skip_nvis, int skip_ld) {
     BVC_REQUIRE(D % 4 == 0, "colsum_f32: D must be a multiple of 4");
+    BVC_REQUIRE(skip_ld == 0 || (skip_nvis >= 0 && skip_nvis < skip_ld), "colsum_f32: bad skip map (%d of %d rows)", skip_nvis, skip_ld);
     const int RB = 256;
     if (options().deterministic) {
         const int nrb = (M + RB - 1) / RB;
         if (nrb <= 0) return BVC_OK;
         float* part = det_scratch((size_t)nrb * D + det_rows_mid_floats(nrb, D), s);
         if (!part) return BVC_ERR_HIP;
-        hipLaunchKernelGGL(colsum_f32_det_kernel, dim3((D + 255) / 256, nrb), dim3(256), 0, s, X, rm, M, D, part, RB);
+        hipLaunchKernelGGL(colsum_f32_det_kernel, dim3((D + 255) / 256, nrb), dim3(256), 0, s, X, rm, M, D, part, RB, skip_nvis, skip_ld);
         BVC_CHECK_HIP(hipGetLastError());
         return launch_det_rows_reduce(part, nrb, D, D, out, out, part + (size_t)nrb * D, s);
     }
-    hipLaunchKernelGGL(colsum_f32_kernel, dim3((D + 255) / 256, (M + RB - 1) / RB), dim3(256), 0, s, X, rm, M, D, out, RB);
+    hipLaunchKernelGGL(colsum_f32_kernel, dim3((D + 255) / 256, (M + RB - 1) / RB), dim3(256), 0, s, X, rm, M, D, out, RB, skip_nvis, skip_ld);
     BVC_CHECK_HIP(hipGetLastError());
     return BVC_OK;
 }
@@ -1439,6 +1487,20 @@
     return BVC_OK;
 }
 
+int launch_head_assemble(const bf16_t* ln_s, const bf16_t* qkv_s, const float* mean_s, const float* rstd_s, const int* dec_idx, bf16_t* ln1o,
+                         bf16_t* qkv, float* mean1, float* rstd1, int B, int L, int Ld, int nvis, int D, int Q, hipStream_t s) {
+    BVC_REQUIRE(B >= 1 && L >= 1 && nvis >= 1 && nvis < Ld && D % 8 == 0 && Q % 8 == 0, "head_assemble: bad shape (B %d, L %d, Ld %d, nvis %d, D %d, Q %d)",
+                B, L, Ld, nvis, D, Q);
+    const int len = (Ld + 7) / 8;
+    const dim3 grid(8 * balanced_grid((B * len + 3) / 4, 512));
+    if (D <= 512 && Q <= 1536)
+        hipLaunchKernelGGL((head_assemble_kernel<1, 3>), grid, dim3(256), 0, s, ln_s, qkv_s, mean_s, rstd_s, dec_idx, ln1o, qkv, mean1, rstd1, B, L, Ld, nvis, D, Q);
+    else
+        hipLaunchKernelGGL((head_assemble_kernel<0, 0>), grid, dim3(256), 0, s, ln_s, qkv_s, mean_s, rstd_s, dec_idx, ln1o, qkv, mean1, rstd1, B, L, Ld, nvis, D, Q);
+    BVC_CHECK_HIP(hipGetLastError());
+    return BVC_OK;
+}
+
 int launch_target_select(const float* h, const int* idx, float* out, int nsets, int B, int Np, int L, int D, float eps, hipStream_t s) {
     BVC_REQUIRE(D % 4 == 0 && D <= kWideChunks * 256, "target_select: D=%d unsupported", D);
     const int rows = nsets * B * Np;
diff --git a/baby-vision-curriculum_amd/csrc/stack.h b/baby-vision-curriculum_amd/csrc/stack.h
--- a/baby-vision-curriculum_amd/csrc/stack.h
+++ b/baby-vision-curriculum_amd/csrc/stack.h
@@ -96,6 +96,17 @@
 struct LayerTail { int nvis, ndec; };
 bool layer_tail_ok(const Work& w, const Stack& s, int B, int nvis, int ndec);
 
+struct LayerHead {
+    int nvis, ndec, L;
+    const int* pos_idx;
+    const float* x_t;
+    bf16_t *ln, *qkv;
+    float *mean, *rstd;
+    float* skip_part;
+    float* dsum;
+};
+bool layer_head_ok(const Work& w, const Stack& s, int B, int nvis, int ndec);
+
 LayerOff add_layer_params(ParamTable& t, const std::string& prefix, int64_t d, int64_t inter, bool hf_names);
 int alloc_stack(Arena& a, Stack& s, int D, int I, int H, int nlayers, float eps, size_t M, size_t BHN);
 int alloc_work(Arena& a, Work& w, size_t MD, size_t MI, size_t delta_elems, size_t lnpart_elems);
@@ -107,7 +118,7 @@
 int join_side(Work& w, int parity, hipStream_t st, bvc_bucket_fn on_bucket, void* user);
 void begin_backward(Work& w);
 int layer_forward(Work& w, Stack& s, int li, const LayerOff& o, const float* x_in, float* x_out, int B, int N, hipStream_t st,
-                  const LayerOff* next = nullptr, const LayerTail* tail = nullptr);
+                  const LayerOff* next = nullptr, const LayerTail* tail = nullptr, const LayerHead* head = nullptr);
 bool fuse_row_ln(const Stack& s, int M);
 int set_drop(DropState& d, const bvc_branch_drop* drop, int samples, const char* who, hipStream_t st);
 int alloc_drop(Arena& a, DropState& d, int nlayers, int max_samples);
@@ -118,6 +129,6 @@
     return &store;
 }
 int layer_backward(Work& w, Stack& s, int li, const LayerOff& o, const float* x_in, float* dres, float* G, int B, int N,
-                   hipStream_t st, bvc_bucket_fn on_bucket, void* user, const LayerTail* tail = nullptr);
+                   hipStream_t st, bvc_bucket_fn on_bucket, void* user, const LayerTail* tail = nullptr, const LayerHead* head = nullptr);
 
 }
diff --git a/baby-vision-curriculum_amd/csrc/stack.hip b/baby-vision-curriculum_amd/csrc/stack.hip
--- a/baby-vision-curriculum_amd/csrc/stack.hip
+++ b/baby-vision-curriculum_amd/csrc/stack.hip
@@ -222,6 +222,13 @@
     return fuse_row_ln(s, B * (nvis + ndec)) && gemm_row_ln_ok(B * ndec, s.D, s.D);
 }
 
+bool layer_head_ok(const Work& w, const Stack& s, int B, int nvis, int ndec) {
+    if (!options().dec_head || B < 1 || nvis < 1 || ndec < 1) return false;
+    if (w.drop != nullptr && w.drop->active) return false;
+    if (s.hdp != s.hd) return false;
+    return fuse_row_ln(s, B * (nvis + ndec));
+}
+
 int alloc_drop(Arena& a, DropState& d, int nlayers, int max_samples) {
     d.nlayers = nlayers;
     d.max_samples = max_samples;
@@ -259,11 +266,12 @@
 }
 
 int layer_forward(Work& w, Stack& s, int li, const LayerOff& o, const float* x_in, float* x_out, int B, int N, hipStream_t st,
-                  const LayerOff* next, const LayerTail* tail) {
+                  const LayerOff* next, const LayerTail* tail, const LayerHead* head) {
     LayerAct& a = s.act[li];
     const int D = s.D, I = s.I, M = B * N;
     const int Mq = tail ? B * tail->ndec : M;
     if (tail) BVC_REQUIRE(next == nullptr && tail->nvis + tail->ndec == N && layer_tail_ok(w, s, B, tail->nvis, tail->ndec), "layer_forward: tail mode is not available for this layer");
+    if (head) BVC_REQUIRE(li == 0 && head->nvis + head->ndec == N && layer_head_ok(w, s, B, head->nvis, head->ndec), "layer_forward: head mode is not available for this layer");
     const float* P = w.params;
     const bf16_t* W = w.wbf;
     const float eps = s.eps;
@@ -271,7 +279,11 @@
     const int gl = w.drop_layer >= 0 ? w.drop_layer : li;
     const bool fuse = !gated && fuse_row_ln(s, M);
     if (li == 0) s.ln1_ready = false;
-    if (!(fuse && s.ln1_ready)) TRY(launch_ln_fwd(x_in, identity_rows(), P + o.ln1w, P + o.ln1b, a.ln1o, a.mean1, a.rstd1, M, D, eps, st));
+    if (head) {
+        const int T = head->L;
+        TRY(launch_ln_fwd(head->x_t, identity_rows(), P + o.ln1w, P + o.ln1b, head->ln, head->mean, head->rstd, T, D, eps, st));
+        TRY(launch_ln_fwd(x_in, RowMap{head->nvis, N, 0}, P + o.ln1w, P + o.ln1b, head->ln + (size_t)T * D, head->mean + T, head->rstd + T, B * head->nvis, D, eps, st));
+    } else if (!(fuse && s.ln1_ready)) TRY(launch_ln_fwd(x_in, identity_rows(), P + o.ln1w, P + o.ln1b, a.ln1o, a.mean1, a.rstd1, M, D, eps, st));
     s.ln1_ready = false;
     const int Da = s.Da;
     const bool pad = s.hdp != s.hd;
@@ -282,7 +294,14 @@
         TRY(launch_pad_heads(W + o.wqkv, P + o.bqkv, W + o.wo, s.wqkv_pad, s.bqkv_pad, s.wo_pad, D, s.H, s.hd, s.hdp, st));
         Wqkv = s.wqkv_pad; Wo = s.wo_pad; bqkv = s.bqkv_pad;
     }
-    {
+    if (head) {
+        const int Mh = head->L + B * head->nvis;
+        GemmProblem p = gemm(head->ln, (size_t)Mh * D, D, Wqkv, (size_t)3 * Da * D, D, Mh, 3 * Da, D, EPI_BF16, head->qkv, 3 * Da);
+        p.bias = bqkv;
+        TRY(launch_gemm(&p, 1, GEMM_NT, -1, st));
+        TRY(launch_head_assemble(head->ln, head->qkv, head->mean, head->rstd, head->pos_idx, a.ln1o, a.qkv, a.mean1, a.rstd1, B, head->L, N, head->nvis,
+                                 D, 3 * Da, st));
+    } else {
         GemmProblem p = gemm(a.ln1o, (size_t)M * D, D, Wqkv, (size_t)3 * Da * D, D, M, 3 * Da, D, EPI_BF16, a.qkv, 3 * Da);
         p.bias = bqkv;
         TRY(launch_gemm(&p, 1, GEMM_NT, -1, st));
@@ -327,7 +346,7 @@
 }
 
 int layer_backward(Work& c_, Stack& s, int li, const LayerOff& o, const float* x_in, float* dres, float* G, int B, int N,
-                   hipStream_t st, bvc_bucket_fn on_bucket, void* user, const LayerTail* tail) {
+                   hipStream_t st, bvc_bucket_fn on_bucket, void* user, const LayerTail* tail, const LayerHead* head) {
     LayerAct& a = s.act[li];
     const int D = s.D, I = s.I, M = B * N;
     const int Mq = tail ? B * tail->ndec : M;
@@ -348,6 +367,7 @@
     if (gated) { g_attn = c_.drop->gate(li, 0); if (li > 0) g_below = c_.drop->gate(li - 1, 1); }
     const bool fuse = !gated && fuse_row_ln(s, M);
     if (tail) BVC_REQUIRE(fuse && tail->nvis + tail->ndec == N, "layer_backward: tail mode needs the row-LayerNorm epilogues");
+    if (head) BVC_REQUIRE(fuse && li == 0 && head->nvis + head->ndec == N && head->skip_part && head->dsum, "layer_backward: head mode needs the row-LayerNorm epilogues of layer 0");
     if (fuse) {
         GemmProblem p = gemm(dh, (size_t)Mq * I, I, W + o.w1, (size_t)I * D, D, Mq, D, I, EPI_DLN, dres, D);
         p.C2 = dhb; p.ln_x = a.h; p.ln_mean = a.mean2; p.ln_rstd = a.rstd2; p.ln_gamma = P + o.ln2w;
@@ -378,7 +398,12 @@
         GemmProblem p = gemm(dqkv, (size_t)M * 3 * Da, 3 * Da, Wqkv, (size_t)3 * Da * D, D, M, D, 3 * Da, EPI_DLN, dres, D);
         p.C2 = dyb_next; p.ln_x = x_in; p.ln_mean = a.mean1; p.ln_rstd = a.rstd1; p.ln_gamma = P + o.ln1w;
         p.ln_part = c_.ln_part; p.ln_dgamma = G + o.ln1w; p.ln_dbeta = G + o.ln1b;
-        TRY(launch_gemm(&p, 1, GEMM_NN, -1, st));
+        if (head) {
+            p.rin = head->nvis; p.rout = N; p.partial = head->skip_part;
+            BVC_CHECK_HIP(hipMemsetAsync(head->skip_part, 0, kRowLnSkipFloats * sizeof(float), st));
+        }
+        TRY(launch_gemm(&p, 1, GEMM_NN, -1, st));
+        if (head) TRY(launch_colsum_f32(head->skip_part, identity_rows(), kRowLnSkipRows, D, head->dsum, st));
     } else {
         GemmProblem p = gemm(dqkv, (size_t)M * 3 * Da, 3 * Da, Wqkv, (size_t)3 * Da * D, D, M, D, 3 * Da, EPI_BF16, c_.dln, D);
         TRY(launch_gemm(&p, 1, GEMM_NN, -1, st));
diff --git a/baby-vision-curriculum_amd/csrc/videomae.hip b/baby-vision-curriculum_amd/csrc/videomae.hip
--- a/baby-vision-curriculum_amd/csrc/videomae.hip
+++ b/baby-vision-curriculum_amd/csrc/videomae.hip
@@ -99,6 +99,10 @@
     float *dres_enc, *dres_dec;
     bf16_t* de2d;
     bool tail_on = false;
+    int* pos_iota;
+    float *head_x, *head_mean, *head_rstd, *head_skip;
+    bf16_t *head_ln, *head_qkv;
+    bool head_on = false;
 };
 
 namespace {
@@ -146,6 +150,7 @@
     else if (!strcmp(name, "deterministic")) { BVC_REQUIRE(value == 0 || value == 1, "set_option: deterministic takes 0 / 1"); options().deterministic = value; }
     else if (!strcmp(name, "head_pad")) { BVC_REQUIRE(value == 0 || value == 1, "set_option: head_pad takes 0 / 1"); options().head_pad = value; }
     else if (!strcmp(name, "dec_tail")) { BVC_REQUIRE(value == 0 || value == 1, "set_option: dec_tail takes 0 / 1"); options().dec_tail = value; }
+    else if (!strcmp(name, "dec_head")) { BVC_REQUIRE(value == 0 || value == 1, "set_option: dec_head takes 0 / 1"); options().dec_head = value; }
     else BVC_REQUIRE(false, "set_option: unknown option '%s'", name);
     return BVC_OK;
 }
@@ -157,6 +162,7 @@
     if (name && !strcmp(name, "deterministic")) return options().deterministic;
     if (name && !strcmp(name, "head_pad")) return options().head_pad;
     if (name && !strcmp(name, "dec_tail")) return options().dec_tail;
+    if (name && !strcmp(name, "dec_head")) return options().dec_head;
     bvc::set_error("get_option: unknown option '%s'", name ? name : "(null)");
     return BVC_ERR_INVALID;
 }
@@ -254,6 +260,17 @@
     A(alloc_stack(c->arena, c->enc, D, I, H, cfg->num_hidden_layers, cfg->layer_norm_eps, Mv, B * H * c->nvis));
     A(alloc_stack(c->arena, c->dec, Dd, Id, Hd, cfg->decoder_num_hidden_layers, cfg->layer_norm_eps, Md, B * Hd * c->Ld));
     A(c->arena.alloc(&c->xe_bf, Mv * D));
+    {
+        const size_t Lp = c->L, Mh = Lp + Mv;
+        A(c->arena.alloc(&c->pos_iota, Lp));
+        A(launch_iota_mod(c->pos_iota, c->L, c->L, nullptr));
+        A(c->arena.alloc(&c->head_x, Lp * Dd));
+        A(c->arena.alloc(&c->head_ln, Mh * Dd));
+        A(c->arena.alloc(&c->head_qkv, Mh * 3 * c->dec.Da));
+        A(c->arena.alloc(&c->head_mean, Mh));
+        A(c->arena.alloc(&c->head_rstd, Mh));
+        A(c->arena.alloc(&c->head_skip, kRowLnSkipFloats));
+    }
     A(c->arena.alloc(&c->meanf, Mm));
     A(c->arena.alloc(&c->rstdf, Mm));
     A(c->arena.alloc(&c->lnf, Mm * Dd));
@@ -331,10 +348,14 @@
     TRY(launch_fill_masked(c->dec.act[0].x_in, params + L.mask_token, c->pos_dec, c->dec_idx, B, Ld, nvis, ndec, Dd, st));
     const LayerTail lt{nvis, ndec};
     c->tail_on = layer_tail_ok(c->w, c->dec, B, nvis, ndec);
+    const LayerHead lh{nvis, ndec, Lq, c->dec_idx, c->head_x, c->head_ln, c->head_qkv, c->head_mean, c->head_rstd, nullptr, nullptr};
+    c->head_on = layer_head_ok(c->w, c->dec, B, nvis, ndec);
+    if (c->head_on) TRY(launch_fill_masked(c->head_x, params + L.mask_token, c->pos_dec, c->pos_iota, 1, Lq, 0, Lq, Dd, st));
     for (int i = 0; i < c->dec.nlayers; ++i) {
         const bool last = i + 1 == c->dec.nlayers;
         float* xo = !last ? c->dec.act[i + 1].x_in : c->dec.x_out;
-        TRY(layer_forward(c->w, c->dec, i, L.dec[i], c->dec.act[i].x_in, xo, B, Ld, st, !last ? &L.dec[i + 1] : nullptr, last && c->tail_on ? &lt : nullptr));
+        TRY(layer_forward(c->w, c->dec, i, L.dec[i], c->dec.act[i].x_in, xo, B, Ld, st, !last ? &L.dec[i + 1] : nullptr, last && c->tail_on ? &lt : nullptr,
+                          i == 0 && c->head_on ? &lh : nullptr));
     }
     const RowMap tail = c->tail_on ? identity_rows() : RowMap{ndec, Ld, nvis};
     TRY(launch_ln_fwd(c->dec.x_out, tail, params + L.norm_w, params + L.norm_b, c->lnf, c->meanf, c->rstdf, Mm, Dd, cf.decoder_norm_eps, st));
@@ -392,11 +413,12 @@
                           G + L.norm_w, G + L.norm_b, c->w.ln_part, Mm, Dd, st));
     }
     bucket(L.norm_w, L.total);
+    const LayerHead lh{nvis, ndec, c->L, c->dec_idx, c->head_x, c->head_ln, c->head_qkv, c->head_mean, c->head_rstd, c->head_skip, G + L.mask_token};
     for (int i = c->dec.nlayers - 1; i >= 0; --i) {
         TRY(layer_backward(c->w, c->dec, i, L.dec[i], c->dec.act[i].x_in, c->dres_dec, G, B, Ld, st, on_bucket, user,
-                           i + 1 == c->dec.nlayers && c->tail_on ? &lt : nullptr));
-    }
-    TRY(launch_colsum_f32(c->dres_dec, tail, Mm, Dd, G + L.mask_token, st));
+                           i + 1 == c->dec.nlayers && c->tail_on ? &lt : nullptr, i == 0 && c->head_on ? &lh : nullptr));
+    }
+    TRY(launch_colsum_f32(c->dres_dec, tail, Mm, Dd, G + L.mask_token, st, c->head_on ? nvis : 0, c->head_on ? Ld : 0));
     const RowMap headrows{nvis, Ld, 0};
     TRY(launch_gather_rows_bf16(c->dres_dec, headrows, c->de2d, Mv, Dd, st));
     {
@@ -946,6 +968,17 @@
     s.hd = width / heads; s.hdp = attn_width(s.hd); s.Da = heads * s.hdp;
     return fuse_row_ln(s, tokens) ? 1 : 0;
 }
+int bvc_op_dec_head_selected(int clips, int visible, int decoded, int width, int mlp_width, int heads, int gated) {
+    if (clips <= 0 || width <= 0 || heads <= 0 || width % heads != 0) return 0;
+    Stack s;
+    s.D = width; s.I = mlp_width; s.H = heads; s.nlayers = 0; s.eps = 0.f; s.x_out = nullptr;
+    s.hd = width / heads; s.hdp = attn_width(s.hd); s.Da = heads * s.hdp;
+    DropState d;
+    d.active = gated != 0;
+    Work w;
+    w.drop = &d;
+    return layer_head_ok(w, s, clips, visible, decoded) ? 1 : 0;
+}
 int bvc_op_sgd_step_segments(float* params, float* grads, float* momentum_buf, int64_t n, const int64_t* seg_start, const int32_t* seg_group,
                              const int32_t* blk_seg, int nseg, const bvc_sgd_groups* groups, const float* grad_scale, const float* found_inf,
                              int write_unscaled_grads, void* bf16_shadow, void* stream) {
diff --git a/baby-vision-curriculum_amd/probe.py b/baby-vision-curriculum_amd/probe.py
--- a/baby-vision-curriculum_amd/probe.py
+++ b/baby-vision-curriculum_amd/probe.py
@@ -34,6 +34,8 @@
         Bm = _rb(dev, N, K) if layout == _ops.NT else _rb(dev, K, N)
         Bm.mul_(0.02)
         kw = {}
+        skip = epi == "DLN_SKIP"
+        epi = "DLN" if skip else epi
         out_f32 = epi in ("F32", "RESID", "POS", "E2D", "F32_BF16", "RESID_LN", "DLN")
         nbytes = 2.0 * (M * K + N * K)
         Mo = M
@@ -61,6 +63,9 @@
                       ln_mean=torch.zeros(M, device=dev), ln_rstd=torch.ones(M, device=dev), ln_part=torch.empty(512 * 2 * N, device=dev),
                       ln_dgamma=torch.zeros(N, device=dev), ln_dbeta=torch.zeros(N, device=dev))
             nbytes += (4.0 + 4.0 + 2.0) * M * N
+            if skip:
+                kw.update(rin=160, rout=1568, partial=torch.zeros(512 * N, device=dev))
+                nbytes -= (4.0 + 2.0) * (M // 1568) * 1312 * N
         if epi == "DGELU":
             kw["aux"] = _rb(dev, M, N)
             nbytes += 2.0 * M * N
@@ -113,7 +118,10 @@
     one("enc fc1+GELU", NT, Mv, I, D, "GELU", 12)
     one("enc fc2", NT, Mv, D, I, "RESID", 12)
     one("enc->dec", NT, Mv, Dd, D, "E2D", 1)
-    one("dec qkv", NT, Md, 3 * Dd, Dd, "BF16", 4)
+    head = bool(_lib.lib().bvc_op_dec_head_selected(B, 160, 1408, Dd, Id, 6, 0))
+    one("dec qkv", NT, Md, 3 * Dd, Dd, "BF16", 3 if head else 4)
+    if head:
+        one("dec qkv, layer 0 (position table + visible rows)", NT, 1568 + Mv, 3 * Dd, Dd, "BF16", 1)
     if fused:
         one("dec proj + LayerNorm", NT, Md, Dd, Dd, "RESID_LN", 4)
     else:
@@ -129,7 +137,9 @@
     one("dec dX fc2", NN, Md, Id, Dd, "DGELU", 4)
     one("dec dX fc1 + LayerNorm bwd" if fused else "dec dX fc1", NN, Md, Dd, Id, "DLN" if fused else "BF16", 4)
     one("dec dX proj", NN, Md, Dd, Dd, "BF16", 4)
-    one("dec dX qkv + LayerNorm bwd" if fused else "dec dX qkv", NN, Md, Dd, 3 * Dd, "DLN" if fused else "BF16", 4)
+    one("dec dX qkv + LayerNorm bwd" if fused else "dec dX qkv", NN, Md, Dd, 3 * Dd, "DLN" if fused else "BF16", 3 if head else 4)
+    if head:
+        one("dec dX qkv + LayerNorm bwd, layer 0 (decoded-only units: column sums, no stores)", NN, Md, Dd, 3 * Dd, "DLN_SKIP", 1)
     one("enc->dec dX", NN, Mv, D, Dd, "F32_BF16", 1)
     one("enc dX fc2", NN, Mv, I, D, "DGELU", 12)
     one("enc dX fc1", NN, Mv, D, I, "BF16", 12)
@@ -171,7 +181,8 @@
     st = _lib.current_stream_ptr
     p = lambda t: ctypes.c_void_p(t.data_ptr())
     fused = bool(lib.bvc_op_row_ln_selected(B * 1568, 384, 1536, 6))
-    for label, M, Dm, count, count_bwd in (("enc", B * 160, 768, 24, 24), ("dec", B * 1568, 384, 1 if fused else 8, 0 if fused else 8),
+    head = bool(lib.bvc_op_dec_head_selected(B, 160, 1408, 384, 1536, 6, 0))
+    for label, M, Dm, count, count_bwd in (("enc", B * 160, 768, 24, 24), ("dec", 1568 + B * 160 if head else B * 1568, 384, 1 if fused else 8, 0 if fused else 8),
                                            ("final", B * 1408, 384, 1, 1)):
         x, dres = torch.randn(M, Dm, device=dev), torch.randn(M, Dm, device=dev)
         gmm, bta = torch.ones(Dm, device=dev), torch.zeros(Dm, device=dev)
diff --git a/include/bvc.h b/include/bvc.h
--- a/include/bvc.h
+++ b/include/bvc.h
@@ -185,6 +185,7 @@
 int bvc_op_gemm_gate_kernel(const bvc_gemm_desc* problem, int tile_cfg, char* name, int name_cap);
 int bvc_op_gemm_kernel(const bvc_gemm_desc* problems, int count, int layout, int tile_cfg, int stages, char* name, int name_cap);
 int bvc_op_row_ln_selected(int tokens, int width, int mlp_width, int heads);
+int bvc_op_dec_head_selected(int clips, int visible, int decoded, int width, int mlp_width, int heads, int gated);
 int bvc_op_gemm_plan_dw(bvc_gemm_desc* problems, int count);
 
 int bvc_op_attention_fwd(const void* qkv, void* ctx_out, float* lse, int B, int N, int H, int head_dim, void* stream);
```

Result: no change. 3287 clips/s, median of 2 (+0.3%).
